# saholmes/stark-mlwe

Measured on AMD Instinct MI355X. Metric: prove ms + Fr-NTT achieved GB/s, 2^20/2^24 trace at 1/2/4/8 GPUs, higher is better.
Workload: dtype u256 (4x u64 Montgomery limbs, Pallas Fr); 1 GPU; one 2^20-row trace x 4 columns (2^20 rows per GPU), blowup 8: LDE (iNTT + coset NTT) + DEEP-ALI merge + FRI folds + Poseidon leaf hashes + Poseidon-Merkle trees (schedule [16,16,8]), kernels only; log_trace_per_gpu=20, log_blowup=3, field=pallas_fr

## Files before the change

### stark_mlwe_amd/csrc/capi_core.hip

```cpp
#include <algorithm>
#include <cstring>
#include "poseidon_launch.hpp"
#include "pow_table.hpp"

using namespace stark;

namespace stark {

static int32_t pool_poison_fill(stark_ctx* ctx, void* p, size_t bytes) {
    STARK_HIP(ctx, hipMemsetAsync(p, ctx->opt.pool_poison, bytes, ctx->stream));
    STARK_HIP(ctx, hipStreamSynchronize(ctx->stream));
    return STARK_OK;
}

int32_t ctx_scratch(stark_ctx* ctx, size_t bytes, void** out) {
    if (bytes > ctx->scratch_bytes) {
        if (ctx->scratch) STARK_HIP(ctx, hipStreamSynchronize(ctx->stream));
        ctx->scratch_bytes = 0; STARK_HIP(ctx, ctx->scratch.alloc(bytes)); ctx->scratch_bytes = bytes;
    }
    if (ctx->opt.pool_poison >= 0 && ctx->scratch_bytes) STARK_TRY(pool_poison_fill(ctx, ctx->scratch.p, ctx->scratch_bytes));
    *out = ctx->scratch.p; return STARK_OK;
}

int32_t ctx_upload_staged(stark_ctx* ctx, void* dst, const void* src, size_t bytes) {
    if (!bytes) return STARK_OK;
    auto& q = ctx->staged;
    for (size_t i = 0; i < q.size();) {
        if (hipEventQuery(q[i].done) == hipSuccess) { (void)hipEventDestroy(q[i].done); q[i] = std::move(q.back()); q.pop_back(); } else ++i;
    }
    (void)hipGetLastError();
    stark_ctx::StagedUpload u; u.host.reset(new uint8_t[bytes]); memcpy(u.host.get(), src, bytes);
    STARK_HIP(ctx, hipEventCreateWithFlags(&u.done, hipEventDisableTiming));
    const uint8_t* from = u.host.get();
    q.push_back(std::move(u));
    STARK_HIP(ctx, hipMemcpyAsync(dst, from, bytes, hipMemcpyHostToDevice, ctx->stream));
    STARK_HIP(ctx, hipEventRecord(q.back().done, ctx->stream));
    return STARK_OK;
}

static inline size_t pool_round(size_t bytes) {
    if (bytes < 256) return 256;
    if (bytes <= (1u << 20)) { size_t r = 256; while (r < bytes) r <<= 1; return r; }
    return (bytes + (1u << 20) - 1) & ~(size_t)((1u << 20) - 1);
}
int32_t ctx_alloc(stark_ctx* ctx, size_t bytes, void** out) {
    const size_t sz = pool_round(bytes);
    auto it = ctx->pool_free.find(sz);
    if (it != ctx->pool_free.end() && !it->second.empty()) {
        void* p = it->second.back(); it->second.pop_back(); ctx->pool_cached_bytes -= sz;
        ctx->pool_live[p] = sz; *out = p;
        return ctx->opt.pool_poison >= 0 ? pool_poison_fill(ctx, p, sz) : STARK_OK;
    }
    void* p = nullptr; hipError_t e = hipMalloc(&p, sz);
    if (e != hipSuccess) {
        (void)hipGetLastError();
        (void)hipStreamSynchronize(ctx->stream);
        for (auto& kv : ctx->pool_free) { for (void* q : kv.second) (void)hipFree(q); kv.second.clear(); }
        ctx->pool_cached_bytes = 0;
        e = hipMalloc(&p, sz);
        if (e != hipSuccess) { (void)hipGetLastError(); return ctx->fail(STARK_ERR_OOM, "device allocation of " + std::to_string(sz) + " bytes failed"); }
    }
    ctx->pool_live[p] = sz; *out = p;
    return ctx->opt.pool_poison >= 0 ? pool_poison_fill(ctx, p, sz) : STARK_OK;
}
void ctx_release(stark_ctx* ctx, void* p) {
    if (!p || !ctx) return;
    auto it = ctx->pool_live.find(p);
    if (it == ctx->pool_live.end()) { ctx->err = "ctx_release: the pointer is not a live block of this context's pool (left alone)"; return; }
    const size_t sz = it->second; ctx->pool_live.erase(it);
    ctx->pool_free[sz].push_back(p); ctx->pool_cached_bytes += sz;
}
int32_t ctx_enter(stark_ctx* ctx) {
    if (!ctx) return STARK_ERR_INVALID_ARG;
    int cur = -1;
    if (hipGetDevice(&cur) != hipSuccess || cur != ctx->device) STARK_HIP(ctx, hipSetDevice(ctx->device));
    return STARK_OK;
}

int32_t ctx_side_stream(stark_ctx* ctx, hipStream_t* out) {
    if (!ctx->side_stream) { STARK_HIP(ctx, hipStreamCreateWithFlags(&ctx->side_stream, hipStreamNonBlocking)); STARK_HIP(ctx, hipEventCreateWithFlags(&ctx->ev_fork, hipEventDisableTiming)); }
    *out = ctx->side_stream; return STARK_OK;
}
int32_t ctx_fork(stark_ctx* ctx, hipStream_t* side) {
    STARK_TRY(ctx_side_stream(ctx, side));
    if (hipEventRecord(ctx->ev_fork, ctx->stream) != hipSuccess || hipStreamWaitEvent(*side, ctx->ev_fork, 0) != hipSuccess) return ctx->fail(STARK_ERR_HIP, "fork");
    return STARK_OK;
}
int32_t ctx_join(stark_ctx* ctx) {
    if (hipEventRecord(ctx->ev_fork, ctx->side_stream) != hipSuccess || hipStreamWaitEvent(ctx->stream, ctx->ev_fork, 0) != hipSuccess) return ctx->fail(STARK_ERR_HIP, "join");
    return STARK_OK;
}

static int32_t params_finish(stark_ctx* ctx, stark_params* P) {
    if (host::rp_for_width(P->ref.t) < 0) return ctx->fail(STARK_ERR_UNSUPPORTED, "Poseidon width must be one of 9,17,33,65,129");
    P->kc = host::make_kernel_consts(P->ref);
    if (!P->kc.ok) return ctx->fail(STARK_ERR_UNSUPPORTED, "MDS matrix has a singular leading minor: LU/sparse kernel form unavailable");
    const host::KernelConsts& k = P->kc;
    std::vector<fr_t> blob; auto put = [&](const std::vector<fr_t>& v) { size_t off = blob.size(); blob.insert(blob.end(), v.begin(), v.end()); return off; };
    size_t o_rcf = put(k.rc_full), o_rcp = put(k.rc_partial), o_lu = put(k.lu), o_pre = put(k.lu_pre), o_row0 = put(k.row0), o_sp = put(k.sparse), o_mds = put(k.mds), o_mpre = put(k.mds_pre), o_gam = put(k.gamma);
    const size_t o_29 = blob.size();
    { std::vector<uint32_t> w29; for (auto* v : {&k.lu29, &k.lu_pre29, &k.row0_29, &k.sparse29, &k.gamma29, &k.mds29, &k.mds_pre29, &k.chain_a, &k.chain_g, &k.chain_w}) w29.insert(w29.end(), v->begin(), v->end());
      while (w29.size() % 8) w29.push_back(0);
      blob.resize(o_29 + w29.size() / 8); memcpy((void*)(blob.data() + o_29), w29.data(), w29.size() * 4); }
    const size_t o_frag = blob.size(), frag_elems = (k.mds_frag.size() + sizeof(fr_t) - 1) / sizeof(fr_t);
    if (!k.mds_frag.empty()) { blob.resize(o_frag + 2 * frag_elems); memcpy((void*)(blob.data() + o_frag), k.mds_frag.data(), k.mds_frag.size()); memcpy((void*)(blob.data() + o_frag + frag_elems), k.mds_pre_frag.data(), k.mds_pre_frag.size()); }
    const size_t o_b8 = blob.size(), ef_elems = (k.blk8_efrag.size() + sizeof(fr_t) - 1) / sizeof(fr_t), lf_elems = (k.blk8_lfrag.size() + sizeof(fr_t) - 1) / sizeof(fr_t), gf_elems = (k.blk8_gfrag.size() + sizeof(fr_t) - 1) / sizeof(fr_t);
    if (!k.blk8_efrag.empty()) { blob.resize(o_b8 + ef_elems + lf_elems + gf_elems); memcpy((void*)(blob.data() + o_b8), k.blk8_efrag.data(), k.blk8_efrag.size()); memcpy((void*)(blob.data() + o_b8 + ef_elems), k.blk8_lfrag.data(), k.blk8_lfrag.size());
                                 memcpy((void*)(blob.data() + o_b8 + ef_elems + lf_elems), k.blk8_gfrag.data(), k.blk8_gfrag.size()); }
    STARK_HIP(ctx, P->blob.alloc(blob.size() * sizeof(fr_t)));
    fr_t* const dev = P->blob.fr();
    STARK_HIP(ctx, hipMemcpyAsync(dev, blob.data(), blob.size() * sizeof(fr_t), hipMemcpyHostToDevice, ctx->stream));
    STARK_HIP(ctx, hipStreamSynchronize(ctx->stream));
    P->dev.t = k.t; P->dev.rf = k.rf; P->dev.rp = k.rp;
    P->dev.rc_full = dev + o_rcf; P->dev.rc_partial = dev + o_rcp; P->dev.lu = dev + o_lu; P->dev.lu_pre = dev + o_pre;
    P->dev.row0 = dev + o_row0; P->dev.sparse = dev + o_sp; P->dev.mds = dev + o_mds; P->dev.mds_pre = dev + o_mpre; P->dev.gamma = dev + o_gam;
    { const uint32_t* b29 = reinterpret_cast<const uint32_t*>(dev + o_29);
      P->dev.lu29 = b29; P->dev.lu_pre29 = b29 + k.lu29.size(); P->dev.row0_29 = P->dev.lu_pre29 + k.lu_pre29.size();
      P->dev.sparse29 = P->dev.row0_29 + k.row0_29.size(); P->dev.gamma29 = P->dev.sparse29 + k.sparse29.size();
      P->dev.mds29 = P->dev.gamma29 + k.gamma29.size(); P->dev.mds_pre29 = P->dev.mds29 + k.mds29.size();
      const uint32_t* ch = P->dev.mds_pre29 + k.mds_pre29.size();
      P->dev.chain_a = k.chain_a.empty() ? nullptr : ch; P->dev.chain_g = k.chain_a.empty() ? nullptr : ch + k.chain_a.size(); P->dev.chain_w = k.chain_a.empty() ? nullptr : ch + k.chain_a.size() + k.chain_g.size(); }
    P->dev.blk8_efrag = k.blk8_efrag.empty() ? nullptr : (const void*)(dev + o_b8); P->dev.blk8_lfrag = k.blk8_efrag.empty() ? nullptr : (const void*)(dev + o_b8 + ef_elems);
    P->dev.blk8_gfrag = k.blk8_gfrag.empty() ? nullptr : (const void*)(dev + o_b8 + ef_elems + lf_elems);
    P->dev.blk8_unit_frag = k.blk8_efrag.empty() ? nullptr : (const void*)((const int8_t*)P->dev.blk8_lfrag + k.blk8_lfrag.size() - 1024);
    P->dev.mds_frag = k.mds_frag.empty() ? nullptr : (const void*)(dev + o_frag); P->dev.mds_pre_frag = k.mds_frag.empty() ? nullptr : (const void*)(dev + o_frag + frag_elems);
    return STARK_OK;
}
static int32_t params_from_consts(stark_ctx* ctx, const host::PoseidonConsts& c, std::unique_ptr<stark_params>& out) {
    std::unique_ptr<stark_params> P(new stark_params()); P->ctx = ctx; P->ref = c;
    STARK_TRY(params_finish(ctx, P.get()));
    out = std::move(P); return STARK_OK;
}
static int32_t params_for_caller(stark_ctx* ctx, const host::PoseidonConsts& c, stark_params** out) {
    std::unique_ptr<stark_params> P; STARK_TRY(params_from_consts(ctx, c, P));
    P->ref_.bind(ctx); *out = P.release(); return STARK_OK;
}
int32_t ctx_transcript_params(stark_ctx* ctx, stark_params** out) {
    if (!ctx->tparams) STARK_TRY(params_from_consts(ctx, host::consts_transcript(), ctx->tparams));
    if (out) *out = ctx->tparams.get();
    return STARK_OK;
}
int32_t ctx_merkle_params(stark_ctx* ctx, int t, stark_params** out) {
    auto it = ctx->merkle_params.find(t);
    if (it == ctx->merkle_params.end()) {
        if (host::rp_for_width(t) < 0) return ctx->fail(STARK_ERR_UNSUPPORTED, "unsupported Poseidon width");
        std::unique_ptr<stark_params> P; STARK_TRY(params_from_consts(ctx, host::consts_for_width(t), P));
        *out = P.get(); ctx->merkle_params[t] = std::move(P); return STARK_OK;
    }
    *out = it->second.get(); return STARK_OK;
}
int32_t ctx_commit_params(stark_ctx* ctx, stark_params** out) {
    std::unique_ptr<stark_params>& slot = ctx->merkle_params[-17];
    if (!slot) STARK_TRY(params_from_consts(ctx, host::derive_consts("POSEIDON-T17-X5-SEED", 17, 8, 64), slot));
    *out = slot.get(); return STARK_OK;
}

}

extern "C" {

int32_t stark_version(void) { return 1; }

int32_t stark_ctx_create(int32_t device, void* stream, stark_ctx_t** out) {
    if (!out) return STARK_ERR_INVALID_ARG;
    int ndev = 0;
    if (hipGetDeviceCount(&ndev) != hipSuccess || ndev <= 0 || device < 0 || device >= ndev) return STARK_ERR_HIP;
    if (hipSetDevice(device) != hipSuccess) return STARK_ERR_HIP;
    std::unique_ptr<stark_ctx> c(new stark_ctx()); c->device = device;
    if (stream == STARK_STREAM_PRIVATE) { if (hipStreamCreateWithFlags(&c->stream, hipStreamNonBlocking) != hipSuccess) return STARK_ERR_HIP; c->own_stream = true; }
    else { c->stream = (hipStream_t)stream; c->own_stream = false; }
    if (hipEventCreate(&c->ev0) != hipSuccess || hipEventCreate(&c->ev1) != hipSuccess) return STARK_ERR_HIP;
    { int cus = 0; if (hipDeviceGetAttribute(&cus, hipDeviceAttributeMultiprocessorCount, device) == hipSuccess && cus > 0) c->num_cus = cus; }
    stark::ntt_set_attrs();
    stark::poseidon_set_attrs();
    *out = c.release(); return STARK_OK;
}
}
static void ctx_teardown(stark_ctx* ctx) {
    (void)hipSetDevice(ctx->device); (void)hipStreamSynchronize(ctx->stream);
    stark::comm_destroy(ctx);
    stark::ntt_plans_free(ctx);
    for (auto& kv : ctx->pool_free) for (void* q : kv.second) (void)hipFree(q);
    for (auto& kv : ctx->pool_live) (void)hipFree(kv.first);
    if (ctx->pinned) (void)hipHostFree(ctx->pinned);
    for (auto& u : ctx->staged) (void)hipEventDestroy(u.done);
    if (ctx->ev0) (void)hipEventDestroy(ctx->ev0); if (ctx->ev1) (void)hipEventDestroy(ctx->ev1);
    if (ctx->side_stream) (void)hipStreamDestroy(ctx->side_stream);
    if (ctx->ev_fork) (void)hipEventDestroy(ctx->ev_fork);
    if (ctx->own_stream) (void)hipStreamDestroy(ctx->stream);
    delete ctx;
}
namespace stark {
void ctx_ref(stark_ctx* c) { ++c->live_handles; }
void ctx_unref(stark_ctx* c) { if (--c->live_handles == 0 && c->destroy_pending) ctx_teardown(c); }
}
extern "C" {
int32_t stark_ctx_destroy(stark_ctx_t* ctx) {
    if (!ctx) return STARK_ERR_INVALID_ARG;
    if (ctx->destroy_pending) return STARK_ERR_INVALID_ARG;
    STARK_TRY(ctx_enter(ctx));
    (void)hipStreamSynchronize(ctx->stream);
    if (ctx->live_handles > 0) { ctx->destroy_pending = true; return STARK_OK; }
    ctx_teardown(ctx); return STARK_OK;
}
int32_t stark_ctx_sync(stark_ctx_t* ctx) { if (!ctx) return STARK_ERR_INVALID_ARG; STARK_TRY(ctx_enter(ctx)); STARK_HIP(ctx, hipStreamSynchronize(ctx->stream)); return STARK_OK; }
int32_t stark_ctx_trim(stark_ctx_t* ctx) {
    if (!ctx) return STARK_ERR_INVALID_ARG; STARK_TRY(ctx_enter(ctx));
    STARK_HIP(ctx, hipStreamSynchronize(ctx->stream));
    for (auto& kv : ctx->pool_free) { for (void* q : kv.second) (void)hipFree(q); kv.second.clear(); }
    ctx->pool_cached_bytes = 0;
    stark::ntt_plans_free(ctx);
    ctx->scratch.reset(); ctx->scratch_bytes = 0;
    return STARK_OK;
}
size_t stark_ctx_cached_bytes(stark_ctx_t* ctx) { return ctx ? ctx->pool_cached_bytes : 0; }
}
struct OptionDef { const char* key; const char* (*set)(stark_ctx::Options&, int64_t); };
static const OptionDef kOptions[] = {
    {"ntt_direct_max_log", [](stark_ctx::Options& o, int64_t v) -> const char* { if (v < 0 || v > 30) return "0..30"; o.ntt_direct_max_log = (int)v; return nullptr; }},
    {"ntt_merged_coset", [](stark_ctx::Options& o, int64_t v) -> const char* { o.ntt_merged_coset = v != 0; return nullptr; }},
    {"ntt_log_tile", [](stark_ctx::Options& o, int64_t v) -> const char* { if (v != -1 && (v < 8 || v > 12)) return "8..12, or -1 for the default"; o.ntt_log_tile_forced = v != -1; o.ntt_log_tile = v == -1 ? 11 : (int)v; return nullptr; }},
    {"ntt_min_waves", [](stark_ctx::Options& o, int64_t v) -> const char* { if (v != 2 && v != 4) return "2 or 4"; o.ntt_min_waves = (int)v; return nullptr; }},
    {"poseidon_lane_only", [](stark_ctx::Options& o, int64_t v) -> const char* { o.poseidon_lane_only = v != 0; return nullptr; }},
    {"sponge_one_wave", [](stark_ctx::Options& o, int64_t v) -> const char* { o.sponge_one_wave = v != 0; return nullptr; }},
    {"sponge_debug", [](stark_ctx::Options& o, int64_t v) -> const char* { o.sponge_debug = (int)v; return nullptr; }},
    {"merkle_node16_pair", [](stark_ctx::Options& o, int64_t v) -> const char* { o.merkle_node16_pair = v != 0; return nullptr; }},
    {"poseidon_block8", [](stark_ctx::Options& o, int64_t v) -> const char* { o.poseidon_block8 = v != 0; return nullptr; }},
    {"fri_side_pair", [](stark_ctx::Options& o, int64_t v) -> const char* { o.fri_side_pair = v != 0; return nullptr; }},
    {"sumcheck_verify_batch_max_slots", [](stark_ctx::Options& o, int64_t v) -> const char* { if (v < 1) return "at least 1"; o.sumcheck_verify_batch_max_slots = (size_t)v; return nullptr; }},
    {"ntt_batch_max_elems", [](stark_ctx::Options& o, int64_t v) -> const char* { if (v < 1 || v > ((int64_t)1 << 28)) return "1..2^28"; o.ntt_batch_max_elems = (size_t)v; return nullptr; }},
    {"prove_batch_max_rows", [](stark_ctx::Options& o, int64_t v) -> const char* { if (v < 1 || v > ((int64_t)1 << 28)) return "1..2^28"; o.prove_batch_max_rows = (size_t)v; return nullptr; }},
    {"mle_log_tile", [](stark_ctx::Options& o, int64_t v) -> const char* { if (v != -1 && (v < 3 || v > 12)) return "3..12, or -1 for the default"; o.mle_log_tile = (int)v; return nullptr; }},
    {"mle_lane_contiguous", [](stark_ctx::Options& o, int64_t v) -> const char* { if (v < -1 || v > 1) return "0 or 1, or -1 for the default"; o.mle_lane_contiguous = (int)v; return nullptr; }},
    {"lagrange_max_partials", [](stark_ctx::Options& o, int64_t v) -> const char* { if (v != -1 && (v < 1 || v > ((int64_t)1 << 28))) return "1..2^28, or -1 for the default"; o.lagrange_max_partials = v == -1 ? (size_t)1 << 21 : (size_t)v; return nullptr; }},
    {"lagrange_wide_acc", [](stark_ctx::Options& o, int64_t v) -> const char* { if (v < -1 || v > 1) return "0 or 1, or -1 for the default"; o.lagrange_wide_acc = (int)v; return nullptr; }},
    {"pool_poison", [](stark_ctx::Options& o, int64_t v) -> const char* { if (v < -1 || v > 255) return "0..255, or -1 for off"; o.pool_poison = (int)v; return nullptr; }},
};
extern "C" {
int32_t stark_ctx_set_option(stark_ctx_t* ctx, const char* key, int64_t value) {
    if (!ctx || !key) return STARK_ERR_INVALID_ARG;
    STARK_TRY(ctx_enter(ctx));
    const std::string k(key);
    const OptionDef* def = nullptr; std::string known;
    for (const OptionDef& d : kOptions) { if (k == d.key) def = &d; known += (known.empty() ? "" : ", ") + std::string(d.key); }
    if (!def) return ctx->fail(STARK_ERR_INVALID_ARG, "unknown option '" + k + "' (" + known + ")");
    if (const char* range = def->set(ctx->opt, value)) return ctx->fail(STARK_ERR_INVALID_ARG, k + ": " + range);
    STARK_HIP(ctx, hipStreamSynchronize(ctx->stream));
    stark::ntt_plans_free(ctx);
    return STARK_OK;
}
const char* stark_last_error(stark_ctx_t* ctx) { return ctx ? ctx->err.c_str() : "null context"; }
int32_t stark_malloc(stark_ctx_t* ctx, size_t bytes, void** dptr) { if (!ctx || !dptr) return STARK_ERR_INVALID_ARG; STARK_TRY(ctx_enter(ctx)); STARK_HIP(ctx, hipMalloc(dptr, bytes ? bytes : 32)); return STARK_OK; }
int32_t stark_free(stark_ctx_t* ctx, void* dptr) { if (!ctx) return STARK_ERR_INVALID_ARG; STARK_TRY(ctx_enter(ctx)); STARK_HIP(ctx, hipStreamSynchronize(ctx->stream)); STARK_HIP(ctx, hipFree(dptr)); return STARK_OK; }
int32_t stark_memcpy_h2d(stark_ctx_t* ctx, void* d, const void* s, size_t bytes) {
    if (!ctx) return STARK_ERR_INVALID_ARG;
    STARK_TRY(ctx_enter(ctx));
    STARK_HIP(ctx, hipMemcpyAsync(d, s, bytes, hipMemcpyHostToDevice, ctx->stream)); STARK_HIP(ctx, hipStreamSynchronize(ctx->stream)); return STARK_OK; }
int32_t stark_memcpy_d2h(stark_ctx_t* ctx, void* d, const void* s, size_t bytes) {
    if (!ctx) return STARK_ERR_INVALID_ARG;
    STARK_TRY(ctx_enter(ctx));
    STARK_HIP(ctx, hipMemcpyAsync(d, s, bytes, hipMemcpyDeviceToHost, ctx->stream)); STARK_HIP(ctx, hipStreamSynchronize(ctx->stream)); return STARK_OK; }
int32_t stark_timer_start(stark_ctx_t* ctx) { if (!ctx) return STARK_ERR_INVALID_ARG; STARK_HIP(ctx, hipEventRecord(ctx->ev0, ctx->stream)); return STARK_OK; }
int32_t stark_timer_stop_ms(stark_ctx_t* ctx, float* ms) {
    if (!ctx || !ms) return STARK_ERR_INVALID_ARG;
    STARK_TRY(ctx_enter(ctx));
    STARK_HIP(ctx, hipEventRecord(ctx->ev1, ctx->stream)); STARK_HIP(ctx, hipEventSynchronize(ctx->ev1)); STARK_HIP(ctx, hipEventElapsedTime(ms, ctx->ev0, ctx->ev1)); return STARK_OK; }

}
#define STARK_DIAG_ITERS 2048
static __global__ void __launch_bounds__(1024) k_diag_mac_rate(uint32_t* out, uint32_t seed) {
    uint32_t a0 = seed + threadIdx.x, a1 = a0 * 3 + 1, a2 = a0 * 5 + 2, a3 = a0 * 7 + 3, a4 = a0 * 9 + 4, a5 = a0 * 11 + 5, a6 = a0 * 13 + 6, a7 = a0 * 15 + 7;
    uint64_t d0 = a0, d1 = a1, d2 = a2, d3 = a3, d4 = a4, d5 = a5, d6 = a6, d7 = a7; const uint32_t b = seed | 1;
#define STARK_DIAG_MAD(i) asm volatile("v_mad_u64_u32 %0, vcc, %1, %2, %0" : "+v"(d##i) : "v"(a##i), "v"(b) : "vcc");
    for (int i = 0; i < STARK_DIAG_ITERS; ++i) { STARK_DIAG_MAD(0) STARK_DIAG_MAD(1) STARK_DIAG_MAD(2) STARK_DIAG_MAD(3) STARK_DIAG_MAD(4) STARK_DIAG_MAD(5) STARK_DIAG_MAD(6) STARK_DIAG_MAD(7) }
#undef STARK_DIAG_MAD
    out[blockIdx.x * blockDim.x + threadIdx.x] = (uint32_t)(d0 ^ d1 ^ d2 ^ d3 ^ d4 ^ d5 ^ d6 ^ d7);
}
extern "C" {
int32_t stark_diag_mac_rate(stark_ctx_t* ctx, double* lane_macs_per_s) {
    if (!ctx || !lane_macs_per_s) return STARK_ERR_INVALID_ARG;
    STARK_TRY(ctx_enter(ctx));
    hipDeviceProp_t prop; STARK_HIP(ctx, hipGetDeviceProperties(&prop, ctx->device));
    const int blocks = prop.multiProcessorCount * 2, threads = 1024;
    DevBuf o; STARK_HIP(ctx, o.alloc(ctx, (size_t)blocks * threads * 4));
    hipLaunchKernelGGL(k_diag_mac_rate, dim3(blocks), dim3(threads), 0, ctx->stream, (uint32_t*)o.p, 12345u);
    STARK_HIP(ctx, hipEventRecord(ctx->ev0, ctx->stream));
    hipLaunchKernelGGL(k_diag_mac_rate, dim3(blocks), dim3(threads), 0, ctx->stream, (uint32_t*)o.p, 12345u);
    STARK_HIP(ctx, hipGetLastError());
    STARK_HIP(ctx, hipEventRecord(ctx->ev1, ctx->stream)); STARK_HIP(ctx, hipEventSynchronize(ctx->ev1));
    float ms = 0; STARK_HIP(ctx, hipEventElapsedTime(&ms, ctx->ev0, ctx->ev1));
    *lane_macs_per_s = (double)blocks * threads * 8.0 * STARK_DIAG_ITERS / (ms * 1e-3);
    return STARK_OK;
}

int32_t stark_poseidon_params_upload(stark_ctx_t* ctx, int32_t t, int32_t rf, int32_t rp, const uint64_t* mds, const uint64_t* rc_full, const uint64_t* rc_partial, stark_params_t** out) {
    if (!ctx || !mds || !rc_full || !rc_partial || !out || t < 2 || rf <= 0 || (rf & 1) || rp <= 0) return ctx ? ctx->fail(STARK_ERR_INVALID_ARG, "bad params") : STARK_ERR_INVALID_ARG;
    STARK_TRY(ctx_enter(ctx));
    host::PoseidonConsts c; c.t = t; c.rf = rf; c.rp = rp;
    c.mds.resize((size_t)t * t); c.rc_full.resize((size_t)rf * t); c.rc_partial.resize(rp);
    for (size_t i = 0; i < c.mds.size(); ++i) c.mds[i] = load_fr(mds + 4 * i);
    for (size_t i = 0; i < c.rc_full.size(); ++i) c.rc_full[i] = load_fr(rc_full + 4 * i);
    for (size_t i = 0; i < c.rc_partial.size(); ++i) c.rc_partial[i] = load_fr(rc_partial + 4 * i);
    return params_for_caller(ctx, c, out);
}
int32_t stark_poseidon_params_for_width(stark_ctx_t* ctx, int32_t t, stark_params_t** out) {
    if (!ctx || !out) return STARK_ERR_INVALID_ARG;
    STARK_TRY(ctx_enter(ctx));
    if (host::rp_for_width(t) < 0) return ctx->fail(STARK_ERR_UNSUPPORTED, "unsupported Poseidon width t; supported t in {9,17,33,65,129}");
    return params_for_caller(ctx, host::consts_for_width(t), out);
}
int32_t stark_poseidon_params_t17_seed(stark_ctx_t* ctx, const uint8_t* seed, size_t n, stark_params_t** out) {
    if (!ctx || !out || (!seed && n)) return STARK_ERR_INVALID_ARG;
    STARK_TRY(ctx_enter(ctx));
    return params_for_caller(ctx, host::derive_consts(std::string((const char*)seed, n), 17, 8, 64), out);
}
int32_t stark_poseidon_params_export(stark_params_t* p, int32_t* t, int32_t* rf, int32_t* rp, uint64_t* mds, uint64_t* rc_full, uint64_t* rc_partial) {
    if (!p) return STARK_ERR_INVALID_ARG;
    if (t) *t = p->ref.t; if (rf) *rf = p->ref.rf; if (rp) *rp = p->ref.rp;
    if (mds) for (size_t i = 0; i < p->ref.mds.size(); ++i) store_fr(mds + 4 * i, p->ref.mds[i]);
    if (rc_full) for (size_t i = 0; i < p->ref.rc_full.size(); ++i) store_fr(rc_full + 4 * i, p->ref.rc_full[i]);
    if (rc_partial) for (size_t i = 0; i < p->ref.rc_partial.size(); ++i) store_fr(rc_partial + 4 * i, p->ref.rc_partial[i]);
    return STARK_OK;
}
int32_t stark_poseidon_params_free(stark_params_t* p) { if (!p) return STARK_ERR_INVALID_ARG; delete p; return STARK_OK; }

}
```

### stark_mlwe_amd/csrc/host_util.hpp

```cpp
#pragma once
#include <cstdint>
#include <cstring>
#include <string>
#include <vector>
#include "fr.hpp"
#include "fr29.hpp"

namespace stark {
namespace host {

struct Blake3 {
    static constexpr uint32_t kIV[8] = {0x6A09E667u, 0xBB67AE85u, 0x3C6EF372u, 0xA54FF53Au, 0x510E527Fu, 0x9B05688Cu, 0x1F83D9ABu, 0x5BE0CD19u};
    enum : uint32_t { F_CHUNK_START = 1, F_CHUNK_END = 2, F_PARENT = 4, F_ROOT = 8 };
    static uint32_t ror(uint32_t x, unsigned n) { return (x >> n) | (x << (32 - n)); }
    static void mix(uint32_t* v, int a, int b, int c, int d, uint32_t x, uint32_t y) {
        v[a] += v[b] + x; v[d] = ror(v[d] ^ v[a], 16); v[c] += v[d]; v[b] = ror(v[b] ^ v[c], 12);
        v[a] += v[b] + y; v[d] = ror(v[d] ^ v[a], 8);  v[c] += v[d]; v[b] = ror(v[b] ^ v[c], 7);
    }
    static void compress(const uint32_t h[8], const uint8_t block[64], uint32_t blen, uint64_t ctr, uint32_t flags, uint32_t out[16]) {
        static const uint8_t sched[7][16] = {
            {0, 1, 2, 3, 4, 5, 6, 7, 8, 9, 10, 11, 12, 13, 14, 15}, {2, 6, 3, 10, 7, 0, 4, 13, 1, 11, 12, 5, 9, 14, 15, 8},
            {3, 4, 10, 12, 13, 2, 7, 14, 6, 5, 9, 0, 11, 15, 8, 1}, {10, 7, 12, 9, 14, 3, 13, 15, 4, 0, 11, 2, 5, 8, 1, 6},
            {12, 13, 9, 11, 15, 10, 14, 8, 7, 2, 5, 3, 0, 1, 6, 4}, {9, 14, 11, 5, 8, 12, 15, 1, 13, 3, 0, 10, 2, 6, 4, 7},
            {11, 15, 5, 0, 1, 9, 8, 6, 14, 10, 2, 12, 3, 4, 7, 13}};
        uint32_t m[16], v[16];
        for (int i = 0; i < 16; ++i) m[i] = (uint32_t)block[4 * i] | (uint32_t)block[4 * i + 1] << 8 | (uint32_t)block[4 * i + 2] << 16 | (uint32_t)block[4 * i + 3] << 24;
        for (int i = 0; i < 8; ++i) v[i] = h[i];
        for (int i = 0; i < 4; ++i) v[8 + i] = kIV[i];
        v[12] = (uint32_t)ctr; v[13] = (uint32_t)(ctr >> 32); v[14] = blen; v[15] = flags;
        for (int r = 0; r < 7; ++r) {
            const uint8_t* s = sched[r];
            mix(v, 0, 4, 8, 12, m[s[0]], m[s[1]]);   mix(v, 1, 5, 9, 13, m[s[2]], m[s[3]]);
            mix(v, 2, 6, 10, 14, m[s[4]], m[s[5]]);  mix(v, 3, 7, 11, 15, m[s[6]], m[s[7]]);
            mix(v, 0, 5, 10, 15, m[s[8]], m[s[9]]);  mix(v, 1, 6, 11, 12, m[s[10]], m[s[11]]);
            mix(v, 2, 7, 8, 13, m[s[12]], m[s[13]]); mix(v, 3, 4, 9, 14, m[s[14]], m[s[15]]);
        }
        for (int i = 0; i < 8; ++i) { out[i] = v[i] ^ v[i + 8]; out[i + 8] = v[i + 8] ^ h[i]; }
    }
    struct Node { uint32_t h[8]; uint8_t block[64]; uint32_t blen; uint64_t ctr; uint32_t flags; };
    static void cv_of(const Node& n, uint32_t extra, uint32_t cv[8]) { uint32_t o[16]; compress(n.h, n.block, n.blen, n.ctr, n.flags | extra, o); memcpy(cv, o, 32); }
    static Node chunk_node(const uint8_t* p, size_t len, uint64_t index) {
        Node n; memcpy(n.h, kIV, 32); n.ctr = index;
        size_t off = 0; bool first = true;
        while (len - off > 64) {
            uint32_t o[16]; compress(n.h, p + off, 64, index, first ? F_CHUNK_START : 0, o); memcpy(n.h, o, 32);
            off += 64; first = false;
        }
        memset(n.block, 0, 64); memcpy(n.block, p + off, len - off); n.blen = (uint32_t)(len - off);
        n.flags = (first ? F_CHUNK_START : 0) | F_CHUNK_END;
        return n;
    }
    static Node subtree(const uint8_t* p, size_t len, uint64_t index) {
        if (len <= 1024) return chunk_node(p, len, index);
        size_t chunks = (len + 1023) / 1024, left = 1; while (left * 2 < chunks) left *= 2;
        Node l = subtree(p, left * 1024, index), r = subtree(p + left * 1024, len - left * 1024, index + left);
        Node n; memcpy(n.h, kIV, 32); n.ctr = 0; n.blen = 64; n.flags = F_PARENT;
        uint32_t a[8], b[8]; cv_of(l, 0, a); cv_of(r, 0, b);
        for (int i = 0; i < 8; ++i) for (int j = 0; j < 4; ++j) { n.block[4 * i + j] = (uint8_t)(a[i] >> (8 * j)); n.block[32 + 4 * i + j] = (uint8_t)(b[i] >> (8 * j)); }
        return n;
    }
    static void hash(const uint8_t* p, size_t len, uint8_t out[32]) {
        Node root = subtree(p, len, 0);
        if (root.flags & F_PARENT) root.ctr = 0;
        uint32_t cv[8]; cv_of(root, F_ROOT, cv);
        for (int i = 0; i < 8; ++i) for (int j = 0; j < 4; ++j) out[4 * i + j] = (uint8_t)(cv[i] >> (8 * j));
    }
};

struct ChaCha12Rng {
    uint32_t st[16]; uint32_t out[16]; unsigned have = 0;
    explicit ChaCha12Rng(const uint8_t seed[32]) {
        st[0] = 0x61707865u; st[1] = 0x3320646eu; st[2] = 0x79622d32u; st[3] = 0x6b206574u;
        for (int i = 0; i < 8; ++i) st[4 + i] = (uint32_t)seed[4 * i] | (uint32_t)seed[4 * i + 1] << 8 | (uint32_t)seed[4 * i + 2] << 16 | (uint32_t)seed[4 * i + 3] << 24;
        st[12] = st[13] = st[14] = st[15] = 0;
    }
    static uint32_t rol(uint32_t x, unsigned n) { return (x << n) | (x >> (32 - n)); }
    void block() {
        uint32_t x[16]; memcpy(x, st, 64);
        auto Q = [&](int a, int b, int c, int d) {
            x[a] += x[b]; x[d] = rol(x[d] ^ x[a], 16); x[c] += x[d]; x[b] = rol(x[b] ^ x[c], 12);
            x[a] += x[b]; x[d] = rol(x[d] ^ x[a], 8);  x[c] += x[d]; x[b] = rol(x[b] ^ x[c], 7); };
        for (int i = 0; i < 6; ++i) { Q(0, 4, 8, 12); Q(1, 5, 9, 13); Q(2, 6, 10, 14); Q(3, 7, 11, 15); Q(0, 5, 10, 15); Q(1, 6, 11, 12); Q(2, 7, 8, 13); Q(3, 4, 9, 14); }
        for (int i = 0; i < 16; ++i) out[i] = x[i] + st[i];
        if (++st[12] == 0) ++st[13];
        have = 16;
    }
    uint32_t next_u32() { if (!have) block(); return out[16 - have--]; }
    uint64_t next_u64() { uint64_t lo = next_u32(), hi = next_u32(); return lo | hi << 32; }
};

typedef PallasFr PF;
inline fr_t h_one() { return fr_one<PF>(); }
inline fr_t h_zero() { return fr_zero<PF>(); }
inline fr_t h_mul(const fr_t& a, const fr_t& b) { return fr_mul<PF>(a, b); }
inline fr_t h_add(const fr_t& a, const fr_t& b) { return fr_add<PF>(a, b); }
inline fr_t h_sub(const fr_t& a, const fr_t& b) { return fr_sub<PF>(a, b); }
inline fr_t h_u64(uint64_t x) { return fr_from_u64<PF>(x); }
inline fr_t h_from_le_bytes_mod_order(const uint8_t* b, size_t n) {
    fr_t acc = h_zero(); const fr_t two32 = h_u64(1ull << 32);
    size_t nw = (n + 3) / 4;
    for (size_t k = nw; k-- > 0;) {
        uint32_t w = 0; for (size_t j = 0; j < 4; ++j) if (4 * k + j < n) w |= (uint32_t)b[4 * k + j] << (8 * j);
        acc = h_add(h_mul(acc, two32), h_u64(w));
    }
    return acc;
}
inline void h_to_bytes_le(const fr_t& a, uint8_t out[32]) {
    fr_t c = fr_to_canonical<PF>(a);
    for (int i = 0; i < 8; ++i) for (int j = 0; j < 4; ++j) out[4 * i + j] = (uint8_t)(c.v[i] >> (8 * j));
}
inline fr_t h_fr_from_hash(const char* tag, const std::vector<uint8_t>& data) {
    std::vector<uint8_t> buf(tag, tag + strlen(tag)); buf.insert(buf.end(), data.begin(), data.end());
    uint8_t d[32]; Blake3::hash(buf.data(), buf.size(), d);
    uint8_t wide[64]; memset(wide, 0, 64); memcpy(wide, d, 32);
    return h_from_le_bytes_mod_order(wide, 64);
}
inline fr_t h_tag(const char* s) {
    size_t n = strlen(s);
    if (n <= 32) { uint8_t le[32] = {0}; memcpy(le, s, n); return h_from_le_bytes_mod_order(le, 32); }
    fr_t acc = h_zero();
    for (size_t off = 0; off < n; off += 32) { uint8_t le[32] = {0}; size_t c = n - off < 32 ? n - off : 32; memcpy(le, s + off, c); acc = h_add(acc, h_from_le_bytes_mod_order(le, 32)); }
    return acc;
}
inline std::vector<fr_t> h_words(const char* s) {
    std::vector<fr_t> out; size_t n = strlen(s);
    for (size_t off = 0; off < n; off += 31) { uint8_t le[32] = {0}; size_t c = n - off < 31 ? n - off : 31; memcpy(le, s + off, c); out.push_back(h_from_le_bytes_mod_order(le, 32)); }
    return out;
}
inline int tr_hash_frame(const char* tag, std::vector<fr_t>& frame) {
    const fr_t AB = h_tag("FSv1-ABSORB-BYTES"), CH = h_tag("FSv1-CHALLENGE");
    frame.clear();
    frame.push_back(AB); for (auto& w : h_words("FRI/FS")) frame.push_back(w);
    frame.push_back(AB); for (auto& w : h_words(tag)) frame.push_back(w);
    const int np = (int)frame.size();
    frame.push_back(CH); frame.push_back(AB); for (auto& w : h_words("out")) frame.push_back(w);
    return np;
}

struct PoseidonConsts {
    int t = 0, rf = 0, rp = 0;
    std::vector<fr_t> mds;
    std::vector<fr_t> rc_full;
    std::vector<fr_t> rc_partial;
};
inline void put64(std::vector<uint8_t>& v, uint64_t x) { for (int j = 0; j < 8; ++j) v.push_back((uint8_t)(x >> (8 * j))); }
inline PoseidonConsts derive_consts(const std::string& seed, int t, int rf, int rp) {
    PoseidonConsts c; c.t = t; c.rf = rf; c.rp = rp;
    c.mds.resize((size_t)t * t); c.rc_full.resize((size_t)rf * t); c.rc_partial.resize(rp);
    for (int i = 0; i < t; ++i) for (int j = 0; j < t; ++j) { std::vector<uint8_t> d; put64(d, i); put64(d, j); d.insert(d.end(), seed.begin(), seed.end()); c.mds[(size_t)i * t + j] = h_fr_from_hash("POSEIDON-MDS", d); }
    for (int r = 0; r < rf; ++r) for (int i = 0; i < t; ++i) { std::vector<uint8_t> d; put64(d, r); put64(d, i); d.insert(d.end(), seed.begin(), seed.end()); c.rc_full[(size_t)r * t + i] = h_fr_from_hash("POSEIDON-RC-FULL", d); }
    for (int r = 0; r < rp; ++r) { std::vector<uint8_t> d; put64(d, r); d.insert(d.end(), seed.begin(), seed.end()); c.rc_partial[r] = h_fr_from_hash("POSEIDON-RC-PART", d); }
    return c;
}
inline int width_for_arity(size_t arity) { return arity <= 8 ? 9 : arity <= 16 ? 17 : arity <= 32 ? 33 : arity <= 64 ? 65 : arity <= 128 ? 129 : -1; }
inline int rp_for_width(int t) { switch (t) { case 9: return 60; case 17: return 64; case 33: return 68; case 65: return 76; case 129: return 84; default: return -1; } }
inline PoseidonConsts consts_for_width(int t) {
    std::string seed = "POSEIDON-PALLAS-T"; for (int j = 0; j < 8; ++j) seed.push_back((char)(((uint64_t)t >> (8 * j)) & 0xff));
    return derive_consts(seed, t, 8, rp_for_width(t));
}
inline PoseidonConsts consts_transcript() { return derive_consts("POSEIDON-T17-X5-TRANSCRIPT", 17, 8, 64); }

struct KernelConsts {
    int t = 0, rf = 0, rp = 0;
    std::vector<fr_t> rc_full, rc_partial;
    std::vector<fr_t> lu, lu_pre;
    std::vector<fr_t> row0;
    std::vector<fr_t> sparse;
    std::vector<fr_t> mds;
    std::vector<fr_t> mds_pre;
    std::vector<fr_t> gamma;
    std::vector<uint32_t> lu29, lu_pre29, row0_29, sparse29, gamma29;
    std::vector<uint32_t> mds29, mds_pre29;
    std::vector<int8_t> mds_frag, mds_pre_frag;
    std::vector<uint32_t> chain_a, chain_g, chain_w;
    std::vector<int8_t> blk8_efrag, blk8_lfrag, blk8_gfrag;
    std::vector<uint32_t> gamma8_29;
    bool ok = false;
};
template <class Pred> inline std::vector<uint32_t> to_radix29(const std::vector<fr_t>& v, Pred scaled) {
    const fr_t k = fr_from_u64<PF>(1ull << FR29_SBOX_SHIFT);
    std::vector<uint32_t> o(v.size() * 9);
    for (size_t i = 0; i < v.size(); ++i) fr29_const_from<PF>(scaled(i) ? fr_mul<PF>(v[i], k) : v[i], &o[9 * i]);
    return o;
}
inline void mfma_frag_of(fr_t g, int8_t* out) {
    const fr_t k256 = fr_from_u64<PF>(256);
    int8_t d[32][32];
    for (int b = 0; b < 32; ++b, g = h_mul(g, k256)) {
        const fr_t c = fr_to_canonical<PF>(g); int cy = 0;
        for (int k = 0; k < 32; ++k) { const int v = (int)((c.v[k >> 2] >> (8 * (k & 3))) & 0xff) + 0x80 + cy; cy = v >> 8; d[b][k] = (int8_t)((v & 0xff) - 0x80); }
    }
    for (int l = 0; l < 64; ++l) for (int j = 0; j < 16; ++j) out[(size_t)l * 16 + j] = d[16 * (l >> 5) + j][l & 31];
}
inline std::vector<int8_t> mfma_frags(const fr_t* mat, int rows, int cols, const fr_t& scale) {
    std::vector<int8_t> out((size_t)rows * cols * 64 * 16, 0);
    for (int i = 0; i < rows; ++i) for (int e = 0; e < cols; ++e) mfma_frag_of(h_mul(mat[(size_t)i * cols + e], scale), &out[((size_t)i * cols + e) * 64 * 16]);
    return out;
}
inline std::vector<int8_t> mfma_frags(const std::vector<fr_t>& mat, int t) { return mfma_frags(mat.data(), t, t, fr_from_u64<PF>(1ull << FR29_SBOX_SHIFT)); }
inline bool mat_inverse(std::vector<fr_t> a, int n, std::vector<fr_t>& inv) {
    inv.assign((size_t)n * n, h_zero()); for (int i = 0; i < n; ++i) inv[(size_t)i * n + i] = h_one();
    for (int c = 0; c < n; ++c) {
        int p = -1; for (int r = c; r < n; ++r) if (!fr_is_zero(a[(size_t)r * n + c])) { p = r; break; }
        if (p < 0) return false;
        if (p != c) for (int k = 0; k < n; ++k) { std::swap(a[(size_t)p * n + k], a[(size_t)c * n + k]); std::swap(inv[(size_t)p * n + k], inv[(size_t)c * n + k]); }
        fr_t pi = fr_inv<PF>(a[(size_t)c * n + c]);
        for (int k = 0; k < n; ++k) { a[(size_t)c * n + k] = h_mul(a[(size_t)c * n + k], pi); inv[(size_t)c * n + k] = h_mul(inv[(size_t)c * n + k], pi); }
        for (int r = 0; r < n; ++r) if (r != c) {
            fr_t f = a[(size_t)r * n + c]; if (fr_is_zero(f)) continue;
            for (int k = 0; k < n; ++k) { a[(size_t)r * n + k] = h_sub(a[(size_t)r * n + k], h_mul(f, a[(size_t)c * n + k])); inv[(size_t)r * n + k] = h_sub(inv[(size_t)r * n + k], h_mul(f, inv[(size_t)c * n + k])); }
        }
    }
    return true;
}
inline bool lu_pack(const std::vector<fr_t>& m, int n, std::vector<fr_t>& lu) {
    lu = m;
    for (int k = 0; k < n; ++k) {
        if (fr_is_zero(lu[(size_t)k * n + k])) return false;
        fr_t pi = fr_inv<PF>(lu[(size_t)k * n + k]);
        for (int i = k + 1; i < n; ++i) {
            fr_t f = h_mul(lu[(size_t)i * n + k], pi); lu[(size_t)i * n + k] = f;
            for (int j = k + 1; j < n; ++j) lu[(size_t)i * n + j] = h_sub(lu[(size_t)i * n + j], h_mul(f, lu[(size_t)k * n + j]));
        }
    }
    return true;
}
inline KernelConsts make_kernel_consts(const PoseidonConsts& c) {
    KernelConsts k; k.t = c.t; k.rf = c.rf; k.rp = c.rp; k.rc_full = c.rc_full; k.rc_partial = c.rc_partial; k.mds = c.mds;
    const int t = c.t, n = t - 1;
    k.row0.assign(c.mds.begin(), c.mds.begin() + t);
    std::vector<fr_t> cur = c.mds;
    k.sparse.assign((size_t)c.rp * (2 * t - 1), h_zero());
    for (int r = c.rp - 1; r >= 0; --r) {
        std::vector<fr_t> hat((size_t)n * n), hinv;
        for (int i = 0; i < n; ++i) for (int j = 0; j < n; ++j) hat[(size_t)i * n + j] = cur[(size_t)(i + 1) * t + (j + 1)];
        if (!mat_inverse(hat, n, hinv)) return k;
        fr_t* sp = &k.sparse[(size_t)r * (2 * t - 1)];
        sp[0] = cur[0];
        for (int j = 0; j < n; ++j) { fr_t acc = h_zero(); for (int q = 0; q < n; ++q) acc = h_add(acc, h_mul(cur[(size_t)0 * t + (q + 1)], hinv[(size_t)q * n + j])); sp[1 + j] = acc; }
        for (int i = 0; i < n; ++i) sp[t + i] = cur[(size_t)(i + 1) * t + 0];
        std::vector<fr_t> nxt((size_t)t * t);
        for (int j = 0; j < t; ++j) nxt[j] = c.mds[j];
        for (int i = 0; i < n; ++i) for (int j = 0; j < t; ++j) { fr_t acc = h_zero(); for (int q = 0; q < n; ++q) acc = h_add(acc, h_mul(hat[(size_t)i * n + q], c.mds[(size_t)(q + 1) * t + j])); nxt[(size_t)(i + 1) * t + j] = acc; }
        cur.swap(nxt);
    }
    if (c.rp % 4) return k;
    k.gamma.assign((size_t)(c.rp / 4) * 6, h_zero());
    for (int b = 0; b < c.rp / 4; ++b)
        for (int q = 1; q < 4; ++q)
            for (int p2 = 0; p2 < q; ++p2) {
                const fr_t* uq = &k.sparse[(size_t)(4 * b + q) * (2 * t - 1)];
                const fr_t* wp = &k.sparse[(size_t)(4 * b + p2) * (2 * t - 1)];
                fr_t acc = h_zero();
                for (int j = 1; j < t; ++j) acc = h_add(acc, h_mul(uq[j], wp[t - 1 + j]));
                k.gamma[(size_t)b * 6 + q * (q - 1) / 2 + p2] = acc;
            }
    if (!lu_pack(c.mds, t, k.lu)) return k;
    if (!lu_pack(cur, t, k.lu_pre)) return k;
    k.mds_pre = cur;
    const auto upper = [t](size_t i) { return (int)(i % t) >= (int)(i / t); };
    const auto all = [](size_t) { return true; };
    const auto a_and_w = [t](size_t i) { const int c = (int)(i % (2 * t - 1)); return c == 0 || c >= t; };
    k.lu29 = to_radix29(k.lu, upper); k.lu_pre29 = to_radix29(k.lu_pre, upper); k.row0_29 = to_radix29(k.row0, all);
    k.sparse29 = to_radix29(k.sparse, a_and_w); k.gamma29 = to_radix29(k.gamma, all);
    k.mds29 = to_radix29(k.mds, all); k.mds_pre29 = to_radix29(k.mds_pre, all);
    if (t == 17) { k.mds_frag = mfma_frags(k.mds, t); k.mds_pre_frag = mfma_frags(k.mds_pre, t); }
    if (t == 17 && c.rp % 8 == 0) {
        const int nb = c.rp / 8, w = 2 * t - 1;
        const fr_t s20 = fr_from_u64<PF>(1ull << FR29_SBOX_SHIFT);
        std::vector<fr_t> g8((size_t)nb * 28, h_zero()), um((size_t)8 * n), wm((size_t)n * 8);
        for (int b = 0; b < nb; ++b) {
            for (int q = 0; q < 8; ++q) for (int j = 1; j < t; ++j) {
                um[(size_t)q * n + (j - 1)] = k.sparse[(size_t)(8 * b + q) * w + j];
                wm[(size_t)(j - 1) * 8 + q] = k.sparse[(size_t)(8 * b + q) * w + t - 1 + j];
            }
            const std::vector<int8_t> ef = mfma_frags(um.data(), 8, n, h_one()), lf = mfma_frags(wm.data(), n, 8, s20);
            k.blk8_efrag.insert(k.blk8_efrag.end(), ef.begin(), ef.end()); k.blk8_lfrag.insert(k.blk8_lfrag.end(), lf.begin(), lf.end());
            for (int q = 1; q < 8; ++q) for (int p2 = 0; p2 < q; ++p2) {
                fr_t acc = h_zero();
                for (int j = 0; j < n; ++j) acc = h_add(acc, h_mul(um[(size_t)q * n + j], wm[(size_t)j * 8 + p2]));
                g8[(size_t)b * 28 + q * (q - 1) / 2 + p2] = acc;
                k.blk8_gfrag.resize(k.blk8_gfrag.size() + 1024); mfma_frag_of(h_mul(acc, s20), &k.blk8_gfrag[k.blk8_gfrag.size() - 1024]);
            }
        }
        k.blk8_lfrag.resize(k.blk8_lfrag.size() + 1024); mfma_frag_of(h_one(), &k.blk8_lfrag[k.blk8_lfrag.size() - 1024]);
        k.gamma8_29 = to_radix29(g8, all);
    }
    if (t == 17 && c.rp == 64) {
        const int rp = c.rp, w = 2 * t - 1;
        const fr_t scale = fr_from_u64<PF>(1ull << 25);
        auto limbs = [&](const fr_t& v, uint32_t* out) { const fr29_t u = fr29_unpack(h_mul(v, scale)); for (int i = 0; i < 9; ++i) out[i] = u.l[i]; };
        k.chain_a.assign((size_t)rp * 64, 0u); k.chain_g.assign((size_t)rp * 9 * 64, 0u); k.chain_w.assign((size_t)rp * (t - 1) * 9, 0u);
        for (int q = 0; q < rp; ++q) {
            uint32_t l[9]; limbs(k.sparse[(size_t)q * w], l);
            for (int i = 0; i < 9; ++i) k.chain_a[(size_t)q * 64 + 16 + i] = l[i];
            for (int j = 1; j < t; ++j) limbs(k.sparse[(size_t)q * w + t - 1 + j], &k.chain_w[((size_t)q * (t - 1) + (j - 1)) * 9]);
        }
        for (int q = 1; q < rp; ++q)
            for (int p2 = 0; p2 < q; ++p2) {
                const fr_t* uq = &k.sparse[(size_t)q * w]; const fr_t* wp = &k.sparse[(size_t)p2 * w];
                fr_t acc = h_zero();
                for (int j = 1; j < t; ++j) acc = h_add(acc, h_mul(uq[j], wp[t - 1 + j]));
                uint32_t l[9]; limbs(acc, l);
                if (q == p2 + 1) { for (int i = 0; i < 9; ++i) k.chain_a[(size_t)p2 * 64 + 32 + i] = l[i]; }
                else for (int i = 0; i < 9; ++i) k.chain_g[((size_t)p2 * 9 + i) * 64 + q] = l[i];
            }
    }
    k.ok = true;
    return k;
}

inline void permute_dense(fr_t* s, const PoseidonConsts& c) {
    const int t = c.t, half = c.rf / 2; std::vector<fr_t> o(t);
    auto mds = [&]() { for (int i = 0; i < t; ++i) { fr_t acc = h_zero(); for (int j = 0; j < t; ++j) acc = h_add(acc, h_mul(c.mds[(size_t)i * t + j], s[j])); o[i] = acc; } for (int i = 0; i < t; ++i) s[i] = o[i]; };
    for (int r = 0; r < half; ++r) { for (int i = 0; i < t; ++i) s[i] = fr_pow5<PF>(h_add(s[i], c.rc_full[(size_t)r * t + i])); mds(); }
    for (int r = 0; r < c.rp; ++r) { s[0] = fr_pow5<PF>(h_add(s[0], c.rc_partial[r])); mds(); }
    for (int r = half; r < c.rf; ++r) { for (int i = 0; i < t; ++i) s[i] = fr_pow5<PF>(h_add(s[i], c.rc_full[(size_t)r * t + i])); mds(); }
}

}
}
```

### stark_mlwe_amd/csrc/hostcheck.cpp

```cpp
#include <algorithm>
#include <atomic>
#include <cstring>
#include <vector>
#include "fr.hpp"
#include "host_util.hpp"
#include "poseidon_dev.hpp"
#include "fri_plan.hpp"
#include "fri_verify.hpp"
#include "fri_verify_batch.hpp"
#include "mfma_digits.hpp"
#include "poseidon_chain.hpp"
#include "fri_batch.hpp"
#include "ntt_batch_plan.hpp"
#include "sumcheck_impl.hpp"
#include "mle_dev.hpp"
#include "merkle_batch.hpp"
#include "lagrange_dev.hpp"

using namespace stark;

static fr_t ld4(const uint64_t* p) { fr_t x; for (int i = 0; i < 4; ++i) { x.v[2 * i] = (uint32_t)p[i]; x.v[2 * i + 1] = (uint32_t)(p[i] >> 32); } return x; }
static void st4(uint64_t* p, const fr_t& x) { for (int i = 0; i < 4; ++i) p[i] = (uint64_t)x.v[2 * i] | ((uint64_t)x.v[2 * i + 1] << 32); }

static int g_alloc_fill = 0;
static std::vector<uint64_t> hc_block(size_t bytes) { std::vector<uint64_t> v((bytes + 7) / 8 + 1); memset(v.data(), g_alloc_fill, v.size() * sizeof(uint64_t)); return v; }
static std::vector<fr_t> hc_fr_block(size_t n) { std::vector<fr_t> v(n); if (n) memset((void*)v.data(), g_alloc_fill, n * sizeof(fr_t)); return v; }

struct HcParams { host::PoseidonConsts ref; host::KernelConsts kc; PoseidonDev dev; };
static void bind(HcParams* P) {
    P->kc = host::make_kernel_consts(P->ref);
    P->dev.t = P->kc.t; P->dev.rf = P->kc.rf; P->dev.rp = P->kc.rp; P->dev.rc_full = P->kc.rc_full.data(); P->dev.rc_partial = P->kc.rc_partial.data();
    P->dev.lu = P->kc.lu.data(); P->dev.lu_pre = P->kc.lu_pre.data(); P->dev.row0 = P->kc.row0.data(); P->dev.sparse = P->kc.sparse.data(); P->dev.mds = P->kc.mds.data(); P->dev.mds_pre = P->kc.mds_pre.data(); P->dev.gamma = P->kc.gamma.data();
    P->dev.lu29 = P->kc.lu29.data(); P->dev.lu_pre29 = P->kc.lu_pre29.data(); P->dev.row0_29 = P->kc.row0_29.data(); P->dev.sparse29 = P->kc.sparse29.data(); P->dev.gamma29 = P->kc.gamma29.data(); P->dev.mds29 = P->kc.mds29.data(); P->dev.mds_pre29 = P->kc.mds_pre29.data();
    P->dev.mds_frag = nullptr; P->dev.mds_pre_frag = nullptr; P->dev.blk8_efrag = nullptr; P->dev.blk8_lfrag = nullptr; P->dev.blk8_unit_frag = nullptr; P->dev.blk8_gfrag = nullptr;
    P->dev.chain_a = P->kc.chain_a.empty() ? nullptr : P->kc.chain_a.data(); P->dev.chain_g = P->kc.chain_g.empty() ? nullptr : P->kc.chain_g.data(); P->dev.chain_w = P->kc.chain_w.empty() ? nullptr : P->kc.chain_w.data();
}

extern "C" {

int hc_set_alloc_fill(int byte) { if (byte < 0 || byte > 255) return -1; const int old = g_alloc_fill; g_alloc_fill = byte; return old; }
int hc_alloc_probe(size_t bytes, uint8_t* out) { const std::vector<uint64_t> v = hc_block(bytes); memcpy(out, v.data(), bytes); return 0; }

int hc_fr_op(int field, int op, const uint64_t* a, const uint64_t* b, uint64_t* out) {
    fr_t x = ld4(a), y = b ? ld4(b) : x, z;
    if (field == 0) {
        switch (op) { case 0: z = fr_add<PallasFr>(x, y); break; case 1: z = fr_sub<PallasFr>(x, y); break; case 2: z = fr_mul<PallasFr>(x, y); break; case 3: z = fr_inv<PallasFr>(x); break;
            case 4: z = fr_from_u64<PallasFr>(a[0]); break; case 5: z = fr_to_canonical<PallasFr>(x); break; case 6: z = fr_root_of_unity<PallasFr>((unsigned)a[0]); break;
            case 7: z = fr_pow_u64<PallasFr>(x, b[0]); break; case 8: z = fr_pow5_r29<PallasFr>(x); break; default: return -1; }
    } else {
        switch (op) { case 0: z = fr_add<Bls12381Fr>(x, y); break; case 1: z = fr_sub<Bls12381Fr>(x, y); break; case 2: z = fr_mul<Bls12381Fr>(x, y); break; case 3: z = fr_inv<Bls12381Fr>(x); break;
            case 4: z = fr_from_u64<Bls12381Fr>(a[0]); break; case 5: z = fr_to_canonical<Bls12381Fr>(x); break; case 6: z = fr_root_of_unity<Bls12381Fr>((unsigned)a[0]); break;
            case 7: z = fr_pow_u64<Bls12381Fr>(x, b[0]); break; case 8: z = fr_pow5_r29<Bls12381Fr>(x); break; default: return -1; }
    }
    st4(out, z); return 0;
}
int hc_wide_dot(const uint64_t* a, const uint64_t* b, size_t n, uint64_t* out) {
    DotAcc d; d.init();
    for (size_t i = 0; i < n; ++i) { uint32_t c[9]; fr29_const_from<PF>(ld4(a + 4 * i), c); d.mac(c, ld4(b + 4 * i)); }
    st4(out, d.finish()); return 0;
}
int hc_wide_dot32(const uint64_t* a, const uint64_t* b, size_t n, uint64_t* out) {
    if (n > 24) return -1;
    fr_wide w; fr_wide_zero(w);
    for (size_t i = 0; i < n; ++i) fr_wide_mac_f<PF>(w, ld4(a + 4 * i), ld4(b + 4 * i));
    st4(out, fr_wide_reduce<PF>(w)); return 0;
}
}
template <class F> static int hc_ntt29_impl(uint64_t* data, int log_b, int inverse, uint64_t* max_limb, uint64_t* max_top) {
    if (log_b < 1 || log_b > 16) return -1;
    const size_t B = (size_t)1 << log_b;
    fr_t w = fr_root_of_unity<F>((unsigned)log_b); if (inverse) w = fr_inv<F>(w);
    const fr_t k32 = fr_from_u64<F>(32);
    std::vector<fr29_t> tw(B / 2), x(B);
    { fr_t acc = k32; for (size_t i = 0; i < B / 2; ++i) { tw[i] = fr29_unpack(acc); acc = fr_mul<F>(acc, w); } }
    uint32_t D[9]; ntt29_offset<F>(D);
    auto brev = [&](size_t v) { size_t r = 0; for (int i = 0; i < log_b; ++i) r |= ((v >> i) & 1) << (log_b - 1 - i); return r; };
    for (size_t p = 0; p < B; ++p) x[brev(p)] = fr29_unpack(ld4(data + 4 * p));
    uint64_t ml = 0, mt = 0;
    const int head = log_b >= 3 ? 3 : log_b;
    {
        const fr29_t w1 = tw[log_b >= 3 ? B >> 3 : 0], w2 = tw[log_b >= 2 ? B >> 2 : 0], w3 = tw[log_b >= 3 ? 3 * (B >> 3) : 0];
        for (size_t g = 0; g < (B >> head); ++g) {
            fr29_t* xs = &x[g << head];
            if (head == 3) ntt29_head<F, 3>(*reinterpret_cast<fr29_t (*)[8]>(xs), w1, w2, w3, D);
            else if (head == 2) ntt29_head<F, 2>(*reinterpret_cast<fr29_t (*)[4]>(xs), w1, w2, w3, D);
            else ntt29_head<F, 1>(*reinterpret_cast<fr29_t (*)[2]>(xs), w1, w2, w3, D);
        }
    }
    for (int s = head + 1; s <= log_b; ++s) {
        const size_t half = (size_t)1 << (s - 1); const bool nrm = ntt29_norm_before(s);
        for (size_t bq = 0; bq < B / 2; ++bq) {
            const size_t j = bq & (half - 1), grp = bq >> (s - 1), i0 = (grp << s) + j, i1 = i0 + half;
            fr29_t a = x[i0], b = x[i1];
            { fr29_t bb = b, aa = a; if (nrm) { fr29_norm(bb); fr29_norm(aa); } for (int k = 0; k < 8; ++k) { ml = std::max<uint64_t>(ml, bb.l[k]); ml = std::max<uint64_t>(ml, aa.l[k]); } mt = std::max<uint64_t>(mt, std::max(bb.l[8], aa.l[8])); }
            ntt29_butterfly<F>(a, b, tw[j << (log_b - s)], D, nrm);
            x[i0] = a; x[i1] = b;
        }
    }
    const bool nrm_out = ntt29_norm_after(log_b);
    fr_t mult = k32; if (inverse) mult = fr_mul<F>(k32, fr_inv<F>(fr_from_u64<F>((uint64_t)B)));
    for (size_t k = 0; k < B; ++k) {
        fr29_t y = x[k];
        for (int i = 0; i < 8; ++i) ml = std::max<uint64_t>(ml, nrm_out ? 0 : y.l[i]);
        if (inverse) {
            if (nrm_out) fr29_norm(y);
            mt = std::max<uint64_t>(mt, y.l[8]);
            const fr29_t r = fr29_mul_mont<F>(fr29_unpack(mult), y);
            st4(data + 4 * k, fr29_pack_reduce<F>(r.l));
        } else {
            fr29_partial_reduce<F>(y);
            st4(data + 4 * k, fr29_pack_reduce<F>(y.l));
        }
    }
    if (max_limb) *max_limb = ml; if (max_top) *max_top = mt;
    return 0;
}
extern "C" {
int hc_partial_reduce(int field, uint32_t* limbs, size_t n) {
    for (size_t i = 0; i < n; ++i) {
        fr29_t x; for (int k = 0; k < 9; ++k) x.l[k] = limbs[9 * i + k];
        if (field == 0) fr29_partial_reduce<PallasFr>(x); else fr29_partial_reduce<Bls12381Fr>(x);
        for (int k = 0; k < 9; ++k) limbs[9 * i + k] = x.l[k];
    }
    return 0;
}
int hc_ntt29(int field, uint64_t* data, int log_b, int inverse, uint64_t* max_limb, uint64_t* max_top) {
    return field == 0 ? hc_ntt29_impl<PallasFr>(data, log_b, inverse, max_limb, max_top) : hc_ntt29_impl<Bls12381Fr>(data, log_b, inverse, max_limb, max_top);
}
int hc_blake3(const uint8_t* p, size_t n, uint8_t* out32) { host::Blake3::hash(p, n, out32); return 0; }
int hc_chacha12_u64s(const uint8_t* seed32, size_t n, uint64_t* out) { host::ChaCha12Rng r(seed32); for (size_t i = 0; i < n; ++i) out[i] = r.next_u64(); return 0; }
int hc_from_le_bytes_mod_order(const uint8_t* b, size_t n, uint64_t* out) { st4(out, host::h_from_le_bytes_mod_order(b, n)); return 0; }
int hc_to_bytes_le(const uint64_t* a, uint8_t* out32) { host::h_to_bytes_le(ld4(a), out32); return 0; }

void* hc_params_new(int kind, int t, const char* seed) {
    HcParams* P = new HcParams();
    P->ref = kind == 0 ? host::consts_for_width(t) : kind == 1 ? host::consts_transcript() : host::derive_consts(seed, 17, 8, 64);
    bind(P); return P;
}
void* hc_params_upload(int t, int rf, int rp, const uint64_t* mds, const uint64_t* rc_full, const uint64_t* rc_partial) {
    if (!mds || !rc_full || !rc_partial || t < 2 || rf <= 0 || (rf & 1) || rp <= 0) return nullptr;
    HcParams* P = new HcParams();
    P->ref.t = t; P->ref.rf = rf; P->ref.rp = rp;
    P->ref.mds.resize((size_t)t * t); P->ref.rc_full.resize((size_t)rf * t); P->ref.rc_partial.resize(rp);
    for (size_t i = 0; i < P->ref.mds.size(); ++i) P->ref.mds[i] = ld4(mds + 4 * i);
    for (size_t i = 0; i < P->ref.rc_full.size(); ++i) P->ref.rc_full[i] = ld4(rc_full + 4 * i);
    for (size_t i = 0; i < P->ref.rc_partial.size(); ++i) P->ref.rc_partial[i] = ld4(rc_partial + 4 * i);
    bind(P); return P;
}
int hc_params_ok(void* h) { return ((HcParams*)h)->kc.ok ? 1 : 0; }
void hc_params_free(void* h) { delete (HcParams*)h; }
int hc_params_export(void* h, uint64_t* mds, uint64_t* rc_full, uint64_t* rc_partial) {
    HcParams* P = (HcParams*)h;
    for (size_t i = 0; i < P->ref.mds.size(); ++i) st4(mds + 4 * i, P->ref.mds[i]);
    for (size_t i = 0; i < P->ref.rc_full.size(); ++i) st4(rc_full + 4 * i, P->ref.rc_full[i]);
    for (size_t i = 0; i < P->ref.rc_partial.size(); ++i) st4(rc_partial + 4 * i, P->ref.rc_partial[i]);
    return 0;
}
int hc_full_round_linear(void* h, int which, int pre, uint64_t* states, size_t n) {
    HcParams* P = (HcParams*)h; const int t = P->dev.t;
    if (t != 17 || P->kc.mds_frag.empty()) return -1;
    std::vector<fr_t> st(t), out(t);
    const std::vector<int8_t>& F = pre ? P->kc.mds_pre_frag : P->kc.mds_frag;
    for (size_t s = 0; s < n; ++s) {
        for (int j = 0; j < t; ++j) st[j] = ld4(states + 4 * (s * t + j));
        if (which == 0) { ArrayState a{st.data()}; apply_lu(a, pre ? P->dev.lu_pre29 : P->dev.lu29, t); out = st; }
        else {
            std::vector<fr_t> xd(t); for (int e = 0; e < t; ++e) xd[e] = recode_signed(st[e]);
            for (int i = 0; i < t; ++i) {
                int32_t S[32];
                for (int r = 0; r < 32; ++r) { int64_t acc = 0;
                    for (int e = 0; e < t; ++e) for (int kh = 0; kh < 2; ++kh) { const int8_t* a = &F[((((size_t)i * t + e) * 64) + (r + 32 * kh)) * 16];
                        const int8_t* b = reinterpret_cast<const int8_t*>(xd[e].v) + 16 * kh; for (int j = 0; j < 16; ++j) acc += (int64_t)a[j] * b[j]; }
                    if (acc > 0x7fffffffll || acc < -0x80000000ll) return -2; S[r] = (int32_t)acc; }
                int32_t lo[16], hi[16];
                for (int reg = 0; reg < 16; ++reg) { const int row = (reg & 3) + 8 * (reg >> 2); lo[reg] = S[row]; hi[reg] = S[row + 4]; }
                int64_t col[9]; for (int k = 0; k < 9; ++k) col[k] = 0;
                mfma_fold_rows(col, lo, hi);
                out[i] = mfma_finish_cols(col);
            }
        }
        for (int j = 0; j < t; ++j) st4(states + 4 * (s * t + j), out[j]);
    }
    return 0;
}
size_t hc_mfma_frag_table(void* h, int pre, int8_t* out, size_t cap) {
    HcParams* P = (HcParams*)h; const std::vector<int8_t>& F = pre ? P->kc.mds_pre_frag : P->kc.mds_frag;
    if (out) memcpy(out, F.data(), std::min(cap, F.size()));
    return F.size();
}
int hc_mfma_finish(const int32_t* sums, size_t n, uint64_t* out) {
    for (size_t s = 0; s < n; ++s) {
        const int32_t* S = sums + 32 * s;
        for (int c = 0; c < 32; ++c) if (S[c] >= (1 << 24) || S[c] <= -(1 << 24)) return -1;
        int32_t lo[16], hi[16];
        for (int reg = 0; reg < 16; ++reg) { const int row = (reg & 3) + 8 * (reg >> 2); lo[reg] = S[row]; hi[reg] = S[row + 4]; }
        int64_t col[9]; for (int k = 0; k < 9; ++k) col[k] = 0;
        mfma_fold_rows(col, lo, hi);
        st4(out + 4 * s, mfma_finish_cols(col));
    }
    return 0;
}
static int blk8_tile_sums(const int8_t* const* frag, const fr_t* xd, int K, int32_t* S) {
    for (int r = 0; r < 32; ++r) { int64_t acc = 0;
        for (int k = 0; k < K; ++k) for (int kh = 0; kh < 2; ++kh) { const int8_t* a = frag[k] + (size_t)(r + 32 * kh) * 16;
            const int8_t* b = reinterpret_cast<const int8_t*>(xd[k].v) + 16 * kh; for (int j = 0; j < 16; ++j) acc += (int64_t)a[j] * b[j]; }
        if (acc >= (1 << 24) || acc <= -(1 << 24)) return -2; S[r] = (int32_t)acc; }
    return 0;
}
static fr_t blk8_finish_sums(const int32_t* S) {
    int32_t lo[16], hi[16];
    for (int reg = 0; reg < 16; ++reg) { const int row = (reg & 3) + 8 * (reg >> 2); lo[reg] = S[row]; hi[reg] = S[row + 4]; }
    int64_t col[9]; for (int k = 0; k < 9; ++k) col[k] = 0;
    mfma_fold_rows(col, lo, hi);
    return mfma_finish_cols(col);
}
static int blk8_tile(const int8_t* const* frag, const fr_t* xd, int K, fr_t& out) { int32_t S[32]; const int rc = blk8_tile_sums(frag, xd, K, S); if (rc) return rc; out = blk8_finish_sums(S); return 0; }
static std::atomic<int32_t> g_blk8_row23_max{0};
int32_t hc_blk8_row23_max(int reset) { return reset ? g_blk8_row23_max.exchange(0) : g_blk8_row23_max.load(); }
int hc_permute_block8(void* h, uint64_t* states, size_t n) {
    HcParams* P = (HcParams*)h; const host::KernelConsts& k = P->kc; const int t = k.t, half = k.rf / 2, W = 2 * t - 1;
    if (t != 17 || k.blk8_efrag.empty() || k.blk8_gfrag.empty() || k.mds_frag.empty()) return -1;
    const int8_t* unit = k.blk8_lfrag.data() + k.blk8_lfrag.size() - 1024;
    std::vector<fr_t> st(t), xd(t), o(t);
    auto full = [&](int r, const std::vector<int8_t>& F) -> int {
        for (int j = 0; j < t; ++j) xd[j] = recode_signed(fr_pow5_r29<PF>(fr_add<PF>(st[j], k.rc_full[(size_t)r * t + j])));
        for (int i = 0; i < t; ++i) { const int8_t* fr[17]; for (int e = 0; e < t; ++e) fr[e] = &F[((size_t)i * t + e) * 1024]; const int rc = blk8_tile(fr, xd.data(), t, o[i]); if (rc) return rc; }
        st = o; return 0; };
    for (size_t s = 0; s < n; ++s) {
        for (int j = 0; j < t; ++j) st[j] = ld4(states + 4 * (s * t + j));
        for (int r = 0; r < half; ++r) { const int rc = full(r, r == half - 1 ? k.mds_pre_frag : k.mds_frag); if (rc) return rc; }
        fr_t s0 = st[0], rec[17], y[8], yd[9], kx[23];
        for (int j = 1; j < t; ++j) rec[j] = recode_signed(st[j]);
        const int nb = k.rp / 8;
        for (int b = 0; b < nb; ++b) {
            const int8_t* ef = k.blk8_efrag.data() + (size_t)b * 8 * 16 * 1024; const int8_t* lf = k.blk8_lfrag.data() + (size_t)b * 16 * 8 * 1024;
            const int8_t* gf = k.blk8_gfrag.data() + (size_t)b * 28 * 1024;
            for (int j = 0; j < 16; ++j) kx[j] = rec[1 + j];
            for (int q = 0; q < 8; ++q) {
                const int8_t* fr[23]; for (int j = 0; j < 16; ++j) fr[j] = ef + ((size_t)q * 16 + j) * 1024;
                for (int p2 = 0; p2 < q; ++p2) { fr[16 + p2] = gf + ((size_t)q * (q - 1) / 2 + p2) * 1024; kx[16 + p2] = yd[p2]; }
                int32_t S[32]; { const int rc = blk8_tile_sums(fr, kx, 16 + q, S); if (rc) return rc; }
                if (q == 7) { int32_t m = 0; for (int c = 0; c < 32; ++c) m = std::max(m, S[c] < 0 ? -S[c] : S[c]);
                              int32_t seen = g_blk8_row23_max.load(); while (m > seen && !g_blk8_row23_max.compare_exchange_weak(seen, m)) {} }
                const fr_t H = blk8_finish_sums(S);
                y[q] = fr_pow5_r29<PF>(fr_add<PF>(s0, k.rc_partial[8 * b + q]));
                yd[q] = recode_signed(y[q]);
                DotAcc acc; acc.init();
                acc.mac(c29(k.sparse29.data(), (size_t)(8 * b + q) * W), y[q]);
                s0 = fr_add<PF>(H, acc.finish());
            }
            for (int j = 1; j < t; ++j) {
                const int8_t* fr[9]; for (int p2 = 0; p2 < 8; ++p2) fr[p2] = lf + ((size_t)(j - 1) * 8 + p2) * 1024; fr[8] = unit;
                yd[8] = rec[j];
                fr_t z; { const int rc = blk8_tile(fr, yd, 9, z); if (rc) return rc; }
                if (b == nb - 1) st[j] = z; else rec[j] = recode_signed(z);
            }
        }
        st[0] = s0;
        for (int r = half; r < k.rf; ++r) { const int rc = full(r, k.mds_frag); if (rc) return rc; }
        for (int j = 0; j < t; ++j) st4(states + 4 * (s * t + j), st[j]);
    }
    return 0;
}
size_t hc_blk8_table(void* h, int which, void* out, size_t cap) {
    HcParams* P = (HcParams*)h; const host::KernelConsts& k = P->kc;
    const void* src = which == 0 ? (const void*)k.blk8_efrag.data() : which == 1 ? (const void*)k.blk8_lfrag.data() : which == 3 ? (const void*)k.blk8_gfrag.data() : (const void*)k.gamma8_29.data();
    const size_t len = which == 0 ? k.blk8_efrag.size() : which == 1 ? k.blk8_lfrag.size() : which == 3 ? k.blk8_gfrag.size() : k.gamma8_29.size() * 4;
    if (out && len) memcpy(out, src, std::min(cap, len));
    return len;
}
int hc_blk8_finish_with_base(void* h, const int32_t* sums, const uint64_t* bases, size_t n, uint64_t* out) {
    HcParams* P = (HcParams*)h; if (P->kc.blk8_lfrag.empty()) return -3;
    const int8_t* unit = P->kc.blk8_lfrag.data() + P->kc.blk8_lfrag.size() - 1024;
    for (size_t s = 0; s < n; ++s) {
        const fr_t bd = recode_signed(ld4(bases + 4 * s)); int32_t U[32], S[32];
        if (blk8_tile_sums(&unit, &bd, 1, U)) return -1;
        for (int c = 0; c < 32; ++c) { const int64_t v = (int64_t)sums[32 * s + c] + U[c]; if (v >= (1 << 24) || v <= -(1 << 24)) return -1; S[c] = (int32_t)v; }
        st4(out + 4 * s, blk8_finish_sums(S));
    }
    return 0;
}
int hc_permute_kernel_form(void* h, uint64_t* states, size_t n) {
    HcParams* P = (HcParams*)h; int t = P->dev.t; std::vector<fr_t> st(t);
    for (size_t i = 0; i < n; ++i) { for (int j = 0; j < t; ++j) st[j] = ld4(states + 4 * (i * t + j)); ArrayState s{st.data()}; permute_core(s, P->dev, false); for (int j = 0; j < t; ++j) st4(states + 4 * (i * t + j), st[j]); }
    return 0;
}
int hc_permute_chain_model(void* h, uint64_t* states, size_t n) {
    HcParams* P = (HcParams*)h; const int t = P->ref.t, half = P->ref.rf / 2; if (!P->dev.chain_a) return -1;
    std::vector<fr_t> st(t), o(t);
    auto dense = [&](const std::vector<fr_t>& M) { for (int i = 0; i < t; ++i) { fr_t acc = host::h_zero(); for (int j = 0; j < t; ++j) acc = host::h_add(acc, host::h_mul(M[(size_t)i * t + j], st[j])); o[i] = acc; } st = o; };
    for (size_t i = 0; i < n; ++i) {
        for (int j = 0; j < t; ++j) st[j] = ld4(states + 4 * (i * t + j));
        for (int r = 0; r < half; ++r) { for (int j = 0; j < t; ++j) st[j] = fr_pow5<PallasFr>(host::h_add(st[j], P->ref.rc_full[(size_t)r * t + j])); dense(r == half - 1 ? P->kc.mds_pre : P->kc.mds); }
        chain_partial_model(st.data(), P->dev);
        for (int r = half; r < P->ref.rf; ++r) { for (int j = 0; j < t; ++j) st[j] = fr_pow5<PallasFr>(host::h_add(st[j], P->ref.rc_full[(size_t)r * t + j])); dense(P->kc.mds); }
        for (int j = 0; j < t; ++j) st4(states + 4 * (i * t + j), st[j]);
    }
    return 0;
}
int hc_row_consts(uint32_t* out14) { const RowConstsHost K = row_consts_host(); for (int i = 0; i < 9; ++i) out14[i] = K.ni[i]; for (int i = 0; i < 5; ++i) out14[9 + i] = K.t[i]; return 0; }
size_t hc_chain_table(void* h, int which, uint32_t* out, size_t cap) {
    HcParams* P = (HcParams*)h; const std::vector<uint32_t>& v = which == 0 ? P->kc.chain_a : which == 1 ? P->kc.chain_g : P->kc.chain_w;
    if (out) for (size_t i = 0; i < v.size() && i < cap; ++i) out[i] = v[i];
    return v.size();
}
int hc_permute_dense(void* h, uint64_t* states, size_t n) {
    HcParams* P = (HcParams*)h; int t = P->ref.t; std::vector<fr_t> st(t);
    for (size_t i = 0; i < n; ++i) { for (int j = 0; j < t; ++j) st[j] = ld4(states + 4 * (i * t + j)); host::permute_dense(st.data(), P->ref); for (int j = 0; j < t; ++j) st4(states + 4 * (i * t + j), st[j]); }
    return 0;
}
}
static void leaf_init(fr_t init[17]) {
    const fr_t AB = host::h_tag("FSv1-ABSORB-BYTES"), CH = host::h_tag("FSv1-CHALLENGE");
    for (int j = 0; j < 17; ++j) init[j] = host::h_zero();
    init[0] = AB; init[1] = host::h_words("FRI/leaf/poseidon")[0]; init[2] = AB; init[3] = host::h_words("FRI/leaf")[0];
    init[6] = CH; init[7] = AB; init[8] = host::h_words("leaf")[0]; init[16] = host::h_tag("FSv1-TRANSCRIPT-INIT");
}
extern "C" {
int hc_leaf_pair(void* tparams, const uint64_t* f, const uint64_t* f_next, size_t n, size_t m, uint64_t* hout) {
    HcParams* P = (HcParams*)tparams;
    fr_t init[17]; leaf_init(init);
    std::vector<fr_t> fv(n), nv(f_next ? (n + m - 1) / m : 0);
    for (size_t i = 0; i < fv.size(); ++i) fv[i] = ld4(f + 4 * i);
    for (size_t i = 0; i < nv.size(); ++i) nv[i] = ld4(f_next + 4 * i);
    const LeafStream L{init, fv.data(), f_next ? nv.data() : nullptr, m, n};
    fr_t st[17];
    for (size_t i = 0; i < n; ++i) { ArrayState s{st}; st4(hout + 4 * i, leaf_pair_body(s, P->dev, L, i)); }
    return 0;
}
int hc_hash_ds_level(void* params, int mode, size_t arity, uint32_t level, uint64_t pos0, uint64_t label, const uint64_t* in0, const uint64_t* in1, size_t n_in, uint64_t* out) {
    HcParams* P = (HcParams*)params;
    std::vector<fr_t> a(n_in), b(in1 ? n_in : 0), st(P->dev.t);
    for (size_t i = 0; i < n_in; ++i) { a[i] = ld4(in0 + 4 * i); if (in1) b[i] = ld4(in1 + 4 * i); }
    const DsStream D = DsStream::make(mode, arity, level, pos0, label, a.data(), in1 ? b.data() : nullptr, n_in);
    for (size_t k = 0; k < D.n_out; ++k) { ArrayState s{st.data()}; st4(out + 4 * k, hash_ds_body(s, P->dev, D, k)); }
    return 0;
}
int hc_tr_hash(void* tparams, const char* tag, const uint64_t* fields, size_t k, size_t n, uint64_t* out) {
    HcParams* P = (HcParams*)tparams;
    std::vector<fr_t> fr; const int np = host::tr_hash_frame(tag, fr);
    std::vector<fr_t> fl(n * k); for (size_t i = 0; i < n * k; ++i) fl[i] = ld4(fields + 4 * i);
    const TrStream T = TrStream::equal(fr.data(), np, (int)fr.size() - np, fl.data(), k, n, host::h_tag("FSv1-TRANSCRIPT-INIT"));
    fr_t st[17];
    for (size_t i = 0; i < n; ++i) { ArrayState s{st}; st4(out + 4 * i, tr_hash_body(s, P->dev, T, i)); }
    return 0;
}
int hc_tr_frame_dims(const char* tag, int* np, int* ns) { std::vector<fr_t> fr; *np = host::tr_hash_frame(tag, fr); *ns = (int)fr.size() - *np; return 0; }
int hc_tr_hash_many(void* tparams, size_t n, const char* const* tags, const uint64_t* const* fields, const size_t* k, uint64_t* out, size_t* launch_order) {
    HcParams* P = (HcParams*)tparams;
    std::vector<std::vector<fr_t>> frames(n), fl(n); std::vector<TrFrameRef> fr(n); std::vector<const fr_t*> fp(n, nullptr);
    for (size_t i = 0; i < n; ++i) {
        const int np = host::tr_hash_frame(tags[i], frames[i]); fr[i] = TrFrameRef{frames[i].data(), np, (int)frames[i].size() - np};
        if (!k[i]) continue;
        if (!fields || !fields[i]) return -1;
        fl[i].resize(k[i]); for (size_t q = 0; q < k[i]; ++q) fl[i][q] = ld4(fields[i] + 4 * q);
        fp[i] = fl[i].data();
    }
    const std::vector<TrStream::Item> items = tr_ragged_items(fr.data(), fp.data(), k, n);
    const TrStream T = tr_ragged_stream(items.data(), n, host::h_tag("FSv1-TRANSCRIPT-INIT"));
    fr_t st[17];
    for (size_t j = 0; j < n; ++j) {
        ArrayState s{st}; size_t slot = n; const fr_t d = tr_hash_body<true>(s, P->dev, T, j, &slot);
        if (slot >= n) return -2;
        st4(out + 4 * slot, d); if (launch_order) launch_order[j] = slot;
    }
    return 0;
}
size_t hc_mixed_prove_groups(size_t B, const size_t* n0, const size_t* schedule, const size_t* sched_off, const size_t* r, size_t* group_of, size_t* order) {
    const std::vector<std::vector<size_t>> G = mixed_prove_groups(B, n0, schedule, sched_off, r);
    size_t pos = 0;
    for (size_t g = 0; g < G.size(); ++g) for (size_t i : G[g]) { group_of[i] = g; order[pos++] = i; }
    return G.size();
}
int hc_hash_stream(void* params, int mode, const uint64_t* a, size_t na, const uint64_t* b, size_t nb, const uint64_t* tag, size_t n, uint64_t* out) {
    HcParams* P = (HcParams*)params;
    std::vector<fr_t> av(n * na), bv(n * nb), st(P->dev.t);
    for (size_t i = 0; i < n * na; ++i) av[i] = ld4(a + 4 * i); for (size_t i = 0; i < n * nb; ++i) bv[i] = ld4(b + 4 * i);
    for (size_t k = 0; k < n; ++k) { ArrayState s{st.data()}; st4(out + 4 * k, hash_stream_body(s, P->dev, mode, av.data(), na, bv.data(), nb, tag ? ld4(tag) : host::h_zero(), k)); }
    return 0;
}

struct HcHasher : TrHasher {
    void* tp; explicit HcHasher(void* p) : tp(p) {}
    int32_t hash(const char* tag, const fr_t* fields, size_t k, size_t n, fr_t* out) override {
        std::vector<uint64_t> in(4 * k * n), o(4 * n);
        for (size_t i = 0; i < k * n; ++i) st4(in.data() + 4 * i, fields[i]);
        int rc = hc_tr_hash(tp, tag, in.data(), k, n, o.data()); if (rc) return rc;
        for (size_t i = 0; i < n; ++i) out[i] = ld4(o.data() + 4 * i);
        return 0;
    }
};
struct HcPlan { FriPlan plan; void* tp; };
void* hc_fri_plan_create(void* tparams, const uint64_t* roots, size_t n0, const size_t* schedule, size_t L, size_t r) {
    std::vector<fr_t> rt(L + 1); for (size_t l = 0; l <= L; ++l) rt[l] = ld4(roots + 4 * l);
    HcPlan* P = new HcPlan(); P->tp = tparams; P->plan.r = r; std::string err;
    if (!P->plan.shape.make(n0, schedule, L, rt.data(), err)) { delete P; return nullptr; }
    HcHasher H(tparams); if (fri_plan_make(P->plan, H)) { delete P; return nullptr; }
    return P;
}
size_t hc_fri_plan_num_requests(void* p) { return ((HcPlan*)p)->plan.req.size(); }
int hc_fri_plan_requests(void* p, uint32_t* kind, uint32_t* which, uint32_t* level, uint64_t* index) {
    auto& rq = ((HcPlan*)p)->plan.req;
    for (size_t i = 0; i < rq.size(); ++i) { kind[i] = rq[i].kind; which[i] = rq[i].which; level[i] = rq[i].level; index[i] = rq[i].index; }
    return 0;
}
size_t hc_fri_plan_assemble(void* p, const uint64_t* values, size_t n_values, uint8_t* buf, size_t cap, size_t* est) {
    HcPlan* P = (HcPlan*)p; if (n_values != P->plan.req.size()) return 0;
    std::vector<fr_t> v(n_values); for (size_t i = 0; i < n_values; ++i) v[i] = ld4(values + 4 * i);
    ReplaySource src(v.data(), v.size()); HcHasher H(P->tp); std::vector<uint8_t> b; size_t e = 0;
    if (assemble_proof(P->plan.shape, P->plan.r, H, src, b, e) || src.pos != v.size()) return 0;
    if (est) *est = e;
    if (buf && cap >= b.size()) memcpy(buf, b.data(), b.size());
    return b.size();
}
void hc_fri_plan_free(void* p) { delete (HcPlan*)p; }

struct HcParamCache {
    std::map<int, HcParams*> mp;
    ~HcParamCache() { for (auto& kv : mp) delete kv.second; }
    HcParams* params(size_t arity) { int t = host::width_for_arity(arity); auto it = mp.find(t); if (it != mp.end()) return it->second; HcParams* P = new HcParams(); P->ref = host::consts_for_width(t); bind(P); mp[t] = P; return P; }
};
static HcParamCache& hc_param_cache() { static HcParamCache c; return c; }
static void run_plan_host(VerifyBatchPlan V, const HcParams* tparams, int32_t* accepted) {
    { std::vector<fr_t> dev = hc_fr_block(V.pool.size()); std::copy(V.pool.begin(), V.pool.begin() + V.n_known, dev.begin()); V.pool.swap(dev); }
    if (V.nl) {
        fr_t init[17]; leaf_init(init);
        const LeafStream LS{init, V.pool.data() + V.leaf_f0, V.pool.data() + V.leaf_f0 + V.nl, 1, V.nl};
        fr_t st[17]; for (size_t j = 0; j < V.nl; ++j) { ArrayState s{st}; V.pool[V.leaf_out0 + j] = leaf_pair_body(s, tparams->dev, LS, j); }
    }
    for (const VerifyBatchPlan::Group& G : V.groups) {
        HcParams* P = hc_param_cache().params((size_t)G.t - 1); std::vector<fr_t> st(P->dev.t);
        const DsGatherStream D{V.hdr.data() + 4 * G.job0, V.off.data() + G.job0, V.idx.data(), V.pool.data(), G.n, G.max_children};
        for (size_t k = 0; k < D.n_out; ++k) { ArrayState s{st.data()}; V.pool[G.out0 + k] = hash_ds_body(s, P->dev, D, k); }
    }
    for (size_t b = 0; b < V.batch; ++b) {
        int32_t acc = V.flag[b];
        for (uint32_t j = V.chk_off[b]; j < V.chk_off[b + 1]; ++j) acc &= fr_eq(V.pool[V.chk[2 * j]], V.pool[V.chk[2 * j + 1]]) ? 1 : 0;
        accepted[b] = acc;
    }
}
int hc_deep_fri_verify_batch(void* tparams, size_t batch, const uint8_t* const* proofs, const size_t* lens, const size_t* schedule, size_t L, size_t r, int32_t* accepted) {
    VerifyBatchPlanner pl; for (size_t b = 0; b < batch; ++b) pl.add(proofs[b], lens[b], schedule, L, r);
    if (!pl.fits_u32()) return -1;
    VerifyBatchPlan V; pl.finish(V);
    run_plan_host(std::move(V), (const HcParams*)tparams, accepted);
    return 0;
}
int hc_deep_fri_verify(void* tparams, const uint8_t* bytes, size_t len, const size_t* schedule, size_t L, size_t r) {
    int32_t acc = 0; const int rc = hc_deep_fri_verify_batch(tparams, 1, &bytes, &len, schedule, L, r, &acc);
    return rc ? rc : acc;
}
size_t hc_verify_batch_groups(size_t batch, const uint8_t* const* proofs, const size_t* lens, const size_t* schedule, size_t L, size_t r, int32_t* t, uint32_t* depth, size_t* n, size_t cap) {
    VerifyBatchPlanner pl; for (size_t b = 0; b < batch; ++b) pl.add(proofs[b], lens[b], schedule, L, r);
    VerifyBatchPlan V; pl.finish(V);
    for (size_t g = 0; g < V.groups.size() && g < cap; ++g) { t[g] = V.groups[g].t; depth[g] = V.groups[g].depth; n[g] = V.groups[g].n; }
    return V.groups.size();
}
int hc_merkle_verify(void* tparams, int pairs, size_t cfg_arity, uint64_t label, const uint64_t* root, const size_t* idx, size_t k, const uint64_t* vals, const uint64_t* cp, const uint8_t* proof, size_t len) {
    (void)tparams;
    const uint64_t none[4] = {0, 0, 0, 0};
    MerkleVerifyPlanner pl; pl.add(cfg_arity, label, root, idx, k, vals, pairs ? (cp ? cp : none) : nullptr, proof, len);
    if (!pl.fits_u32()) return -1;
    VerifyBatchPlan V; pl.finish(V);
    int32_t acc = 0; run_plan_host(std::move(V), nullptr, &acc);
    return acc;
}

}

struct ScHostExec {
    HcParams* cp; HcParams* tp; std::vector<std::vector<uint64_t>> mem;
    int32_t alloc(size_t bytes, void** out) { mem.push_back(hc_block(bytes)); *out = mem.back().data(); return 0; }
    int32_t upload(void* dst, const void* src, size_t bytes) { memcpy(dst, src, bytes); return 0; }
    int32_t download(void* dst, const void* src, size_t bytes) { memcpy(dst, src, bytes); return 0; }
    int32_t ds_level(const DsBatchStream& D, fr_t* out) {
        std::vector<fr_t> st(cp->dev.t);
        for (size_t k = 0; k < D.n_out; ++k) { ArrayState s{st.data()}; out[k] = hash_ds_body(s, cp->dev, D, k); }
        return 0;
    }
    int32_t coeffs(const fr_t* const* ptrs, const fr_t* layers, size_t len, size_t B, fr_t* c01, fr_t* claim) {
        for (size_t b = 0; b < B; ++b) {
            const fr_t* l = ptrs ? ptrs[b] : layers + b * len; fr_t c0 = fr_zero<PF>(), c1 = fr_zero<PF>();
            for (size_t j = 0; j < len / 2; ++j) { c0 = fr_add<PF>(c0, l[2 * j]); c1 = fr_add<PF>(c1, fr_sub<PF>(l[2 * j + 1], l[2 * j])); }
            c01[2 * b] = c0; c01[2 * b + 1] = c1; if (claim) claim[b] = fr_add<PF>(fr_add<PF>(c0, c0), c1);
        }
        return 0;
    }
    int32_t fold(const fr_t* const* ptrs, const fr_t* layers, size_t len, size_t B, const fr_t* r, fr_t* next) {
        for (size_t b = 0; b < B; ++b) {
            const fr_t* l = ptrs ? ptrs[b] : layers + b * len;
            for (size_t j = 0; j < len / 2; ++j) next[b * (len / 2) + j] = fr_add<PF>(l[2 * j], fr_mul<PF>(r[b], fr_sub<PF>(l[2 * j + 1], l[2 * j])));
        }
        return 0;
    }
    int32_t transcript(const TrBatchStream& T) { fr_t st[17]; for (size_t a = 0; a < T.n_active; ++a) { ArrayState s{st}; tr_batch_body(s, tp->dev, T, a); } return 0; }
    int32_t gather(const fr_t* const* addr, size_t n, fr_t* out) { for (size_t j = 0; j < n; ++j) out[j] = *addr[j]; return 0; }
};
extern "C" {
int hc_hash_ds_batch_level(void* params, size_t arity, uint32_t level, uint64_t pos0, const uint64_t* labels, const uint64_t* in, size_t n_in, size_t trees, int by_ptrs, uint64_t* out) {
    HcParams* P = (HcParams*)params;
    std::vector<fr_t> a(n_in * trees), st(P->dev.t); for (size_t i = 0; i < a.size(); ++i) a[i] = ld4(in + 4 * i);
    std::vector<const fr_t*> ptrs(trees); for (size_t b = 0; b < trees; ++b) ptrs[b] = a.data() + b * n_in;
    const DsBatchStream D = DsBatchStream::make(arity, level, pos0, labels, by_ptrs ? ptrs.data() : nullptr, by_ptrs ? nullptr : a.data(), n_in, trees);
    for (size_t k = 0; k < D.n_out; ++k) { ArrayState s{st.data()}; st4(out + 4 * k, hash_ds_body(s, P->dev, D, k)); }
    return 0;
}
int hc_tr_batch(void* tparams, uint64_t* state, uint32_t* pos, size_t n_inst, const uint32_t* inst, size_t inst0, size_t n_active, size_t nseg, const uint32_t* el_off,
                const uint32_t* idx, const uint64_t* pool0, size_t n0, const uint64_t* pool1, size_t n1, int reset, int finish_last, uint64_t* out) {
    HcParams* P = (HcParams*)tparams;
    std::vector<fr_t> st(17 * n_inst), p0(n0), p1(n1), o(n_active * nseg, host::h_zero());
    for (size_t i = 0; i < st.size(); ++i) st[i] = ld4(state + 4 * i);
    for (size_t i = 0; i < n0; ++i) p0[i] = ld4(pool0 + 4 * i); for (size_t i = 0; i < n1; ++i) p1[i] = ld4(pool1 + 4 * i);
    TrBatchStream T; T.state = st.data(); T.pos = pos; T.inst = inst; T.inst0 = inst0; T.n_active = n_active; T.nseg = nseg; T.el_off = el_off; T.idx = idx;
    T.pool0 = p0.data(); T.pool1 = p1.data(); T.out = o.data(); T.init_cap = host::h_tag("FSv1-TRANSCRIPT-INIT"); T.reset = reset; T.finish_last = finish_last;
    fr_t s17[17]; for (size_t a = 0; a < n_active; ++a) { ArrayState s{s17}; tr_batch_body(s, P->dev, T, a); }
    for (size_t i = 0; i < st.size(); ++i) st4(state + 4 * i, st[i]);
    for (size_t i = 0; i < o.size(); ++i) st4(out + 4 * i, o[i]);
    return 0;
}
size_t hc_sumcheck_prove_batch(void* tparams, void* cparams, int mf, size_t B, const uint64_t* const* witnesses, size_t k, const uint64_t* labels, size_t q,
                               uint8_t* buf, size_t cap, size_t* lens) {
    const size_t n = (size_t)1 << k;
    std::vector<std::vector<fr_t>> w(B, std::vector<fr_t>(n)); std::vector<const fr_t*> wp(B);
    for (size_t b = 0; b < B; ++b) { for (size_t i = 0; i < n; ++i) w[b][i] = ld4(witnesses[b] + 4 * i); wp[b] = w[b].data(); }
    ScHostExec X{(HcParams*)cparams, (HcParams*)tparams, {}};
    ScBatch<ScHostExec> S(X, B, wp.data(), k, labels);
    std::vector<std::vector<uint8_t>> pr;
    if (mf ? S.prove_mf(q, pr) : S.prove_plain(pr)) return 0;
    size_t tot = 0; for (size_t b = 0; b < B; ++b) { lens[b] = pr[b].size(); tot += pr[b].size(); }
    if (buf && cap >= tot) { size_t o = 0; for (auto& p : pr) { memcpy(buf + o, p.data(), p.size()); o += p.size(); } }
    return tot;
}
}

static int sc_verify_plan(int mf, size_t batch, const uint8_t* const* proofs, const size_t* lens, const uint64_t* labels, ScVerifyPlan& V) {
    bool fits = false;
    if (sc_verify_plan_some(mf, 0, batch, proofs, lens, labels, (size_t)-1, V, fits) != batch || !fits) return -1;
    return 0;
}
extern "C" {
int hc_sc_decode_fr(const uint8_t* blob, size_t len, size_t off, uint64_t* out4) {
    if (off + 32 > len) return -1;
    std::vector<uint32_t> w((len + 3) / 4 + 2, 0u); memcpy(w.data(), blob, len);
    fr_t x; const bool ok = sc_decode_fr(w.data(), (uint32_t)off, 0u, x); st4(out4, x); return ok ? 1 : 0;
}
int hc_sumcheck_verify_batch(void* tparams, void* cparams, int mf, size_t batch, const uint8_t* const* proofs, const size_t* lens, const uint64_t* labels, int32_t* accepted) {
    ScVerifyPlan V; if (sc_verify_plan(mf, batch, proofs, lens, labels, V)) return -1;
    HcParams *tp = (HcParams*)tparams, *cp = (HcParams*)cparams;
    std::vector<fr_t> pool = hc_fr_block(std::max<size_t>(V.pool_slots, 1));
    for (size_t j = 0; j < V.n_dec; ++j) if (!sc_decode_fr(V.blob.data(), V.dec_off[j], V.dec_proof[j], pool[j])) V.flag[V.dec_proof[j] & ~kScClaim] = 0;
    std::vector<fr_t> state = hc_fr_block(17 * std::max<size_t>(V.n_inst, 1)); std::vector<uint32_t> pos(std::max<size_t>(V.n_inst, 1), 0x01010101u * (uint32_t)g_alloc_fill);
    for (const ScVerifyPlan::Stream& S : V.tr) {
        TrBatchStream T; T.state = state.data(); T.pos = pos.data(); T.inst = nullptr; T.inst0 = S.inst0; T.n_active = S.n; T.nseg = S.nseg; T.el_off = V.tr_off.data() + S.seg0;
        T.idx = V.tr_idx.data(); T.pool0 = pool.data(); T.pool1 = V.consts.data(); T.out = pool.data() + V.n_dec + S.seg0; T.init_cap = host::h_tag("FSv1-TRANSCRIPT-INIT"); T.reset = 1; T.finish_last = 1;
        fr_t st[17]; for (size_t a = 0; a < S.n; ++a) { ArrayState s{st}; tr_batch_body(s, tp->dev, T, a); }
    }
    for (const VerifyBatchPlan::Group& G : V.ds.groups) {
        std::vector<fr_t> st(cp->dev.t);
        const DsGatherStream D{V.ds.hdr.data() + 4 * G.job0, V.ds.off.data() + G.job0, V.ds.idx.data(), pool.data(), G.n, G.max_children};
        for (size_t k = 0; k < D.n_out; ++k) { ArrayState s{st.data()}; pool[G.out0 + k] = hash_ds_body(s, cp->dev, D, k); }
    }
    for (size_t j = 0; j < V.n_rec(); ++j) {
        const uint32_t* r = V.rec.data() + 8 * j;
        if (!(mf ? sc_check_mf(pool.data(), r) : sc_check_plain(pool.data(), r))) V.flag[mf ? r[1] : r[0]] = 0;
    }
    for (size_t b = 0; b < batch; ++b) accepted[b] = V.flag[b];
    return 0;
}
size_t hc_sumcheck_verify_batch_steps(int mf, size_t batch, const uint8_t* const* proofs, const size_t* lens, const uint64_t* labels, int32_t* kind, size_t* count, size_t cap) {
    ScVerifyPlan V; if (sc_verify_plan(mf, batch, proofs, lens, labels, V)) return 0;
    const auto st = V.steps();
    for (size_t i = 0; i < st.size() && i < cap; ++i) { kind[i] = st[i].first; count[i] = st[i].second; }
    return st.size();
}
}

struct FriHostExec {
    HcParams* tp; std::vector<std::vector<uint64_t>> mem;
    HcParamCache& mp;
    explicit FriHostExec(HcParams* t) : tp(t), mp(hc_param_cache()) {}
    int32_t alloc(size_t bytes, void** out) { mem.push_back(hc_block(bytes)); *out = mem.back().data(); return 0; }
    int32_t upload(void* dst, const void* src, size_t bytes) { memcpy(dst, src, bytes); return 0; }
    int32_t zpows(const fr_t& z, size_t m, fr_t* zp) { fr_t acc = fr_one<PF>(); for (size_t t = 0; t < m; ++t) { zp[t] = acc; acc = fr_mul<PF>(acc, z); } return 0; }
    int32_t fold(const fr_t* f, size_t n, const fr_t* zp, size_t m, fr_t* out) {
        for (size_t b = 0; b < n / m; ++b) { fr_t acc = fr_zero<PF>(); for (size_t t = 0; t < m; ++t) acc = fr_add<PF>(acc, fr_mul<PF>(f[b * m + t], zp[t])); out[b] = acc; }
        return 0;
    }
    int32_t leaf_pairs(const fr_t* f, const fr_t* f_next, size_t n, size_t m, fr_t* h) {
        fr_t init[17]; leaf_init(init); const LeafStream LS{init, f, f_next, m, n};
        fr_t st[17]; for (size_t i = 0; i < n; ++i) { ArrayState s{st}; h[i] = leaf_pair_body(s, tp->dev, LS, i); }
        return 0;
    }
    template <class DS> int32_t ds(size_t arity, const DS& D, fr_t* out) {
        HcParams* P = mp.params(arity); std::vector<fr_t> st(P->dev.t);
        for (size_t k = 0; k < D.n_out; ++k) { ArrayState s{st.data()}; out[k] = hash_ds_body(s, P->dev, D, k); }
        return 0;
    }
    int32_t pair_level(size_t arity, const DsBatchPairStream& D, fr_t* out) { return ds(arity, D, out); }
    int32_t ds_level(size_t arity, const DsBatchStream& D, fr_t* out) { return ds(arity, D, out); }
    int32_t fork() { return 0; }
    void side(bool) {}
    int32_t join() { return 0; }
};
extern "C" {
int hc_hash_ds_batch_pairs_level(void* params, size_t arity, const uint64_t* labels, const uint64_t* f, const uint64_t* cp, size_t n, size_t cp_div, size_t trees, uint64_t* out) {
    HcParams* P = (HcParams*)params;
    if (!cp_div || n % cp_div) return -1;
    std::vector<fr_t> a(n * trees), b(cp ? n / cp_div * trees : 0), st(P->dev.t);
    for (size_t i = 0; i < a.size(); ++i) a[i] = ld4(f + 4 * i);
    for (size_t i = 0; i < b.size(); ++i) b[i] = ld4(cp + 4 * i);
    const DsBatchPairStream D = DsBatchPairStream::make(arity, labels, a.data(), cp ? b.data() : nullptr, n, cp_div, trees);
    for (size_t k = 0; k < D.n_out; ++k) { ArrayState s{st.data()}; st4(out + 4 * k, hash_ds_body(s, P->dev, D, k)); }
    return 0;
}
int hc_fri_commit_batch(void* tparams, size_t B, const uint64_t* const* f0, size_t n0, const size_t* schedule, size_t L, uint64_t seed_z, uint64_t* roots) {
    FriHostExec X((HcParams*)tparams); FriBatchCommit<FriHostExec> C(X);
    std::string err; if (int rc = C.shape(B, n0, schedule, L, err)) return rc;
    HcHasher H(tparams); std::vector<fr_t> z(L);
    for (size_t l = 0; l < L; ++l) {
        const fr_t in[3] = {host::h_u64(seed_z), host::h_u64(l), host::h_u64(C.n[l])}; fr_t fused; if (H.hash("FRI/z/l", in, 3, 1, &fused)) return -3;
        z[l] = fri_z_from_fused(fused, seed_z, l, C.n[l]);
    }
    if (int rc = C.init(z.data())) return rc;
    for (size_t b = 0; b < B; ++b) for (size_t i = 0; i < n0; ++i) C.f[0][b * n0 + i] = ld4(f0[b] + 4 * i);
    if (int rc = C.run()) return rc;
    for (size_t b = 0; b < B; ++b) for (size_t l = 0; l <= L; ++l) st4(roots + 4 * (b * (L + 1) + l), C.roots[l * B + b]);
    return 0;
}
}

extern "C" {
size_t hc_ntt_batch_passes(size_t batch, int log_out, size_t max_elems, size_t* out, size_t cap) {
    const std::vector<size_t> p = ntt_batch_passes(batch, log_out, max_elems);
    for (size_t i = 0; i < p.size() && i < cap; ++i) out[i] = p[i];
    return p.size();
}
int hc_ntt_batch_ranges_overlap(const uint64_t* starts, size_t batch, size_t bytes) {
    std::vector<const void*> p(batch); for (size_t i = 0; i < batch; ++i) p[i] = (const void*)(uintptr_t)starts[i];
    return ntt_batch_ranges_overlap(p.data(), batch, bytes) ? 1 : 0;
}
}

template <int C>
static void mle_pass_host(bool contig, size_t B, const fr_t* const* ptrs, const fr_t* layers, uint64_t len, int t, const fr_t* r, size_t k, size_t j0, fr_t* next) {
    const int x = t - C; const uint64_t blocks = ((len >> C) + 255) / 256;
    for (size_t b = 0; b < B; ++b) {
        const fr_t* layer = ptrs ? ptrs[b] : layers + b * len; const fr_t* rr = r + b * k + j0; fr_t* dst = next + b * (len >> t);
        for (uint64_t blk = 0; blk < blocks; ++blk) {
            fr_t v[256], u[256]; MleLane L[256]; bool live[256];
            for (int tid = 0; tid < 256; ++tid) {
                L[tid] = mle_lane(blk * 256 + tid, t, C, contig); live[tid] = L[tid].first < len;
                v[tid] = live[tid] ? mle_fold_local<C>(layer + L[tid].first, L[tid].stride, rr + L[tid].local0) : fr_zero<PF>();
            }
            for (int s = 0; s < 6 && s < x; ++s) {
                for (int tid = 0; tid < 256; ++tid) u[tid] = mle_fold1(v[tid], v[tid ^ (1 << s)], rr[L[tid].cross0 + s]);
                std::copy(u, u + 256, v);
            }
            if (x <= 6) { for (int tid = 0; tid < 256; ++tid) if (live[tid] && (tid & ((1 << x) - 1)) == 0) dst[L[tid].tile] = v[tid]; continue; }
            const fr_t w[4] = {v[0], v[64], v[128], v[192]};
            for (int tid = 0; tid < (4 >> (x - 6)); ++tid) {
                const uint64_t tile = (blk << (kMleLogThreads - x)) + tid;
                if ((tile << t) < len) dst[tile] = mle_fold_waves(w, x, tid, rr[L[tid].cross0 + 6], x == 8 ? rr[L[tid].cross0 + 7] : fr_zero<PF>());
            }
        }
    }
}
extern "C" {
int hc_mle_evaluate_batch(size_t B, const uint64_t* const* tables, size_t k, const uint64_t* r, int log_tile, int contig, uint64_t* out, size_t* passes) {
    const int T = log_tile < 0 ? kMleDefaultLogTile : log_tile;
    if (T < kMleMinLogTile || T > kMleMaxLogTile || k > 40) return -1;
    const bool cg = (contig < 0 ? kMleDefaultContig : contig) != 0;
    const std::vector<int> rounds = mle_pass_rounds(k, T);
    if (passes) *passes = rounds.size();
    std::vector<std::vector<fr_t>> tab(B, std::vector<fr_t>((size_t)1 << k)); std::vector<const fr_t*> ptrs(B); std::vector<fr_t> rv(B * k);
    for (size_t b = 0; b < B; ++b) { for (size_t i = 0; i < tab[b].size(); ++i) tab[b][i] = ld4(tables[b] + 4 * i); ptrs[b] = tab[b].data(); }
    for (size_t i = 0; i < rv.size(); ++i) rv[i] = ld4(r + 4 * i);
    if (k == 0) { for (size_t b = 0; b < B; ++b) st4(out + 4 * b, tab[b][0]); return 0; }
    std::vector<fr_t> cur, nxt; size_t j0 = 0;
    for (size_t i = 0; i < rounds.size(); ++i) {
        const int t = rounds[i]; const uint64_t len = (uint64_t)1 << (k - j0);
        nxt = hc_fr_block(B * (len >> t));
        switch (mle_local_rounds(t)) {
            case 0: mle_pass_host<0>(cg, B, i ? nullptr : ptrs.data(), cur.data(), len, t, rv.data(), k, j0, nxt.data()); break;
            case 1: mle_pass_host<1>(cg, B, i ? nullptr : ptrs.data(), cur.data(), len, t, rv.data(), k, j0, nxt.data()); break;
            case 2: mle_pass_host<2>(cg, B, i ? nullptr : ptrs.data(), cur.data(), len, t, rv.data(), k, j0, nxt.data()); break;
            case 3: mle_pass_host<3>(cg, B, i ? nullptr : ptrs.data(), cur.data(), len, t, rv.data(), k, j0, nxt.data()); break;
            case 4: mle_pass_host<4>(cg, B, i ? nullptr : ptrs.data(), cur.data(), len, t, rv.data(), k, j0, nxt.data()); break;
            default: return -1;
        }
        cur.swap(nxt); j0 += (size_t)t;
    }
    for (size_t b = 0; b < B; ++b) st4(out + 4 * b, cur[b]);
    return 0;
}
}
extern "C" int hc_mle_default_log_tile() { return kMleDefaultLogTile; }

struct LagHostExec {
    std::vector<std::vector<uint64_t>> mem; std::vector<fr_t> lo, hi;
    int32_t alloc(size_t bytes, void** out) { mem.push_back(hc_block(bytes)); *out = mem.back().data(); return 0; }
    template <class T> int32_t put(const std::vector<T>& h, T** out) {
        void* p = nullptr; alloc(std::max<size_t>(h.size(), 1) * sizeof(T), &p);
        if (!h.empty()) memcpy(p, h.data(), h.size() * sizeof(T));
        *out = (T*)p; return 0;
    }
    int32_t pow_table(const fr_t& omega, size_t n, LagPow* out) {
        int bits, lo_bits, hi_bits; lag_pow_split(n, &bits, &lo_bits, &hi_bits);
        lo.assign((size_t)1 << lo_bits, fr_one<PF>()); hi.assign((size_t)1 << hi_bits, fr_one<PF>());
        for (size_t i = 1; i < lo.size(); ++i) lo[i] = fr_mul<PF>(lo[i - 1], omega);
        const fr_t step = fr_pow_u64<PF>(omega, (uint64_t)1 << lo_bits);
        for (size_t i = 1; i < hi.size(); ++i) hi[i] = fr_mul<PF>(hi[i - 1], step);
        *out = LagPow{lo.data(), hi.data(), lo_bits}; return 0;
    }
    int32_t gather(const fr_t* const* cols, size_t ncols, const uint64_t* j, const uint64_t* slot, size_t cnt, fr_t* out) {
        for (size_t q = 0; q < cnt; ++q) for (size_t c = 0; c < ncols; ++c) out[slot[q] * ncols + c] = cols[c][j[q]];
        return 0;
    }
    int32_t partials(const fr_t* const* cols, size_t ncols, size_t n, const LagPow& wp, const fr_t& w_step, const fr_t& w_step_inv, const fr_t* zs, size_t npts, unsigned groups, unsigned grid, fr_t* part) {
        const uint32_t T = grid * 256, n32 = (uint32_t)n;
        std::vector<fr_t> Wv(256 * kLagK), w(256), run(256), lane(256);
        auto W = [&](int t) -> fr_t (&)[kLagK] { return *reinterpret_cast<fr_t (*)[kLagK]>(&Wv[(size_t)t * kLagK]); };
        for (unsigned g = 0; g < groups; ++g) for (unsigned blk = 0; blk < grid; ++blk) {
            for (int t = 0; t < 256; ++t) { const uint32_t tid = blk * 256 + t; w[t] = tid < n32 ? lag_pow(wp, tid) : fr_one<PF>(); }
            for (size_t p = g; p < npts; p += groups) {
                const fr_t z = zs[p];
                for (int t = 0; t < 256; ++t) run[t] = lag_prefix(z, w[t], w_step, blk * 256 + (uint32_t)t, T, n32, W(t));
                fr_t tot[4], P = fr_one<PF>();
                for (int v = 0; v < 4; ++v) { tot[v] = fr_one<PF>(); for (int l = 0; l < 64; ++l) tot[v] = fr_mul<PF>(tot[v], run[64 * v + l]); P = fr_mul<PF>(P, tot[v]); }
                const fr_t Pinv = fr_inv<PF>(P);
                for (int t = 0; t < 256; ++t) {
                    const int v = t >> 6, l = t & 63; fr_t before = fr_one<PF>(), after = fr_one<PF>();
                    for (int q = 0; q < l; ++q) before = fr_mul<PF>(before, run[64 * v + q]);
                    for (int q = l + 1; q < 64; ++q) after = fr_mul<PF>(after, run[64 * v + q]);
                    lag_peel(z, w[t], w_step_inv, blk * 256 + (uint32_t)t, T, n32, lag_lane_inverse(Pinv, tot, v, fr_mul<PF>(before, after)), W(t));
                }
                for (size_t c = 0; c < ncols; ++c) {
                    for (int t = 0; t < 256; ++t) lane[t] = lag_lane_dot<kLagWideAcc>(cols[c], blk * 256 + (uint32_t)t, T, n32, W(t));
                    fr_t w4[4];
                    for (int v = 0; v < 4; ++v) { w4[v] = fr_zero<PF>(); for (int l = 0; l < 64; ++l) w4[v] = fr_add<PF>(w4[v], lane[64 * v + l]); }
                    part[(p * ncols + c) * grid + blk] = lag_sum4(w4);
                }
            }
        }
        return 0;
    }
    int32_t finish(const fr_t* part, unsigned grid, const fr_t* scale, const uint64_t* slot, size_t npts, size_t ncols, fr_t* out) {
        for (size_t b = 0; b < npts * ncols; ++b) {
            const size_t p = b / ncols, c = b % ncols; fr_t lane[256];
            for (int t = 0; t < 256; ++t) { lane[t] = fr_zero<PF>(); for (size_t i = (size_t)t; i < grid; i += 256) lane[t] = fr_add<PF>(lane[t], part[b * grid + i]); }
            fr_t w4[4];
            for (int w = 0; w < 4; ++w) { w4[w] = fr_zero<PF>(); for (int l = 0; l < 64; ++l) w4[w] = fr_add<PF>(w4[w], lane[64 * w + l]); }
            out[slot[p] * ncols + c] = fr_mul<PF>(lag_sum4(w4), scale[p]);
        }
        return 0;
    }
};
extern "C" {
int hc_lagrange_eval_batch(size_t ncols, const uint64_t* const* cols, size_t n, const uint64_t* omega, size_t npoints, const uint64_t* z, size_t max_partials, uint64_t* out, size_t* passes) {
    if (passes) *passes = 0;
    if (!ncols || !npoints) return 0;
    if (!n || (n & (n - 1)) || n > ((size_t)1 << kLagMaxLogN)) return -1;
    int lg = 0; while (((size_t)1 << lg) < n) ++lg;
    const fr_t w = omega ? ld4(omega) : fr_root_of_unity<PF>((unsigned)lg);
    if (lag_check_domain(n, w)) return -1;
    std::vector<std::vector<fr_t>> col(ncols, std::vector<fr_t>(n)); std::vector<const fr_t*> ptrs(ncols); std::vector<fr_t> zs(npoints);
    for (size_t c = 0; c < ncols; ++c) {
        size_t first = c; for (size_t q = 0; q < c; ++q) if (cols[q] == cols[c]) { first = q; break; }
        if (first == c) for (size_t i = 0; i < n; ++i) col[c][i] = ld4(cols[c] + 4 * i);
        ptrs[c] = col[first].data();
    }
    for (size_t p = 0; p < npoints; ++p) zs[p] = ld4(z + 4 * p);
    std::vector<fr_t> o = hc_fr_block(npoints * ncols);
    LagHostExec X;
    if (lagrange_eval_batch(X, ncols, ptrs.data(), n, w, npoints, zs.data(), max_partials ? max_partials : kLagDefaultMaxPartials, o.data(), passes)) return -1;
    for (size_t i = 0; i < o.size(); ++i) st4(out + 4 * i, o[i]);
    return 0;
}
}

struct MerkleHostExec {
    HcParams* p; std::vector<std::vector<uint64_t>> mem; std::vector<uint64_t> labels; std::vector<const fr_t*> lv, cpv;
    int32_t level_block(size_t n_fr, fr_t** out) {
        mem.emplace_back(4 * n_fr + 1, g_alloc_fill ? 0x0101010101010101ull * (uint64_t)g_alloc_fill : 0xA5A5A5A5A5A5A5A5ull); *out = (fr_t*)mem.back().data(); return 0;
    }
    int32_t tables(const uint64_t* l, const fr_t* const* leaves, const fr_t* const* cp, size_t B, const uint64_t** lx, const fr_t* const** vx, const fr_t* const** cx) {
        labels.assign(l, l + B); lv.assign(leaves, leaves + B); if (cp) cpv.assign(cp, cp + B);
        *lx = labels.data(); *vx = lv.data(); *cx = cp ? cpv.data() : nullptr; return 0;
    }
    int32_t copy_rows(const fr_t* const* src, size_t n, size_t B, fr_t* dst) { for (size_t b = 0; b < B; ++b) for (size_t i = 0; i < n; ++i) dst[b * n + i] = src[b][i]; return 0; }
    template <class DS> int32_t ds(const DS& D, fr_t* out) {
        std::vector<fr_t> st(p->dev.t);
        for (size_t k = 0; k < D.n_out; ++k) { ArrayState s{st.data()}; out[k] = hash_ds_body(s, p->dev, D, k); }
        return 0;
    }
    int32_t pair_level(const DsBatchPairPtrStream& D, fr_t* out) { return ds(D, out); }
    int32_t ds_level(const DsBatchStream& D, fr_t* out) { return ds(D, out); }
};
struct MerkleOpenHostExec { int32_t gather(const MerkleGatherList& G, fr_t* out) { for (size_t i = 0; i < G.size(); ++i) out[G.row_of(i)] = G.base[G.src[i]][G.index[i]]; return 0; } };
static std::vector<size_t> total_lens(const std::vector<size_t>& lens, size_t B) { std::vector<size_t> o(lens.size() + 1, 0); for (size_t v = 0; v < lens.size(); ++v) o[v + 1] = o[v] + B * lens[v]; return o; }
extern "C" {
int hc_merkle_build_batch(void* params, size_t arity, size_t B, const uint64_t* labels, const uint64_t* const* leaves, size_t n, int pairs, const uint64_t* const* cp,
                          uint64_t* out, size_t cap_fr, size_t* lens_out) {
    HcParams* P = (HcParams*)params;
    if (!B || !n || !arity || host::width_for_arity(arity) != P->dev.t || (arity == 1 && n > 1) || (pairs && !cp)) return -1;
    std::vector<std::vector<fr_t>> col(B, std::vector<fr_t>(n)), cc(B); std::vector<const fr_t*> lp(B), cpp(B, nullptr);
    for (size_t b = 0; b < B; ++b) {
        for (size_t i = 0; i < n; ++i) col[b][i] = ld4(leaves[b] + 4 * i);
        lp[b] = col[b].data();
        if (pairs && cp[b]) { cc[b].resize(n); for (size_t i = 0; i < n; ++i) cc[b][i] = ld4(cp[b] + 4 * i); cpp[b] = cc[b].data(); }
    }
    MerkleHostExec X{P, {}, {}, {}, {}}; std::vector<size_t> lens; std::vector<fr_t*> base;
    if (merkle_build_batch(X, arity, B, labels, lp.data(), n, pairs, pairs ? cpp.data() : nullptr, lens, base)) return -1;
    const std::vector<size_t> at = total_lens(lens, B);
    if (lens.size() > 64 || at.back() > cap_fr) return -1;
    for (size_t v = 0; v < lens.size(); ++v) { lens_out[v] = lens[v]; for (size_t i = 0; i < B * lens[v]; ++i) st4(out + 4 * (at[v] + i), base[v][i]); }
    return (int)lens.size();
}
long hc_merkle_open_batch(size_t B, const size_t* arity, const size_t* nlev, const uint64_t* const* levels, const size_t* lens, const size_t* idx, const size_t* idx_off,
                          uint8_t* buf, size_t cap, size_t* out_lens) {
    std::vector<std::vector<std::vector<fr_t>>> lv(B); std::vector<std::vector<const fr_t*>> lp(B); std::vector<std::vector<size_t>> ll(B); std::vector<MerkleTreeView> views(B);
    for (size_t b = 0, q = 0; b < B; ++b) {
        for (size_t v = 0; v < nlev[b]; ++v, ++q) {
            lv[b].emplace_back(lens[q]); for (size_t i = 0; i < lens[q]; ++i) lv[b][v][i] = ld4(levels[q] + 4 * i);
            ll[b].push_back(lens[q]);
        }
        for (auto& l : lv[b]) lp[b].push_back(l.data());
        views[b] = MerkleTreeView{arity[b], &ll[b], lp[b].data()};
    }
    MerkleOpenHostExec X; std::vector<std::vector<uint8_t>> pr;
    if (merkle_open_batch(X, views.data(), B, idx, idx_off, pr)) return -1;
    size_t tot = 0; for (size_t b = 0; b < B; ++b) { out_lens[b] = pr[b].size(); tot += pr[b].size(); }
    if (buf && cap >= tot) { size_t o = 0; for (auto& p : pr) { memcpy(buf + o, p.data(), p.size()); o += p.size(); } }
    return (long)tot;
}
int hc_merkle_verify_batch(size_t cfg_arity, size_t batch, const uint64_t* labels, const uint64_t* roots, const size_t* indices, const size_t* idx_off, const uint64_t* values,
                           const uint8_t* const* proofs, const size_t* lens, size_t max_slots, int32_t* accepted) {
    if (host::width_for_arity(cfg_arity) < 0 || cfg_arity == 0) return -1;
    auto run = [](const VerifyBatchPlan& V, int32_t* acc) { run_plan_host(V, nullptr, acc); return 0; };
    return merkle_verify_batch(run, cfg_arity, batch, labels, roots, indices, idx_off, values, proofs, lens, max_slots ? max_slots : (size_t)1 << 25, accepted);
}
}
```

### stark_mlwe_amd/csrc/mfma_digits.hpp

```cpp
#pragma once
#include "fr.hpp"
#include "fr29.hpp"

namespace stark {

FR_HD fr_t recode_signed(const fr_t& x) {
    fr_t y; uint64_t c = 0;
#pragma unroll
    for (int i = 0; i < 8; ++i) { const uint64_t t = (uint64_t)x.v[i] + 0x80808080u + c; y.v[i] = (uint32_t)t ^ 0x80808080u; c = t >> 32; }
    return y;
}
template <class V> FR_HD void mfma_fold_rows(int64_t* col, const V& lo, const V& hi) {
#pragma unroll
    for (int q = 0; q < 4; ++q)
#pragma unroll
        for (int hh = 0; hh < 2; ++hh)
#pragma unroll
            for (int p = 0; p < 2; ++p) {
                const V& a = hh ? hi : lo;
                const int64_t pair = (int64_t)a[4 * q + 2 * p] + (int64_t)a[4 * q + 2 * p + 1] * 256;
                const int c = 8 * q + 4 * hh + 2 * p, k = (8 * c) / 29, sh = 8 * c - 29 * k;
                col[k] += pair * ((int64_t)1 << sh);
            }
}
FR_HD fr_t mfma_finish_cols(int64_t* col) {
    typedef PallasFr PF;
    static_assert(fr_p29<PF>(4) < (1u << 10) && fr_p29<PF>(5) == 0 && fr_p29<PF>(6) == 0 && fr_p29<PF>(7) == 0 && fr_p29<PF>(8) == (1u << 22), "r = 2^254 + t with t below 2^126");
    uint32_t l[9];
#pragma unroll
    for (int k = 0; k < 8; ++k) { col[k + 1] += col[k] >> 29; l[k] = (uint32_t)col[k] & FR_M29; }
    const int64_t top = col[8];
    const int32_t q1 = (int32_t)(top >> 22) - 1;
    l[8] = ((uint32_t)top & ((1u << 22) - 1)) + (1u << 22);
    int64_t carry = 0;
#pragma unroll
    for (int i = 0; i < 5; ++i) { const int64_t d = (int64_t)l[i] - (int64_t)q1 * (int64_t)fr_p29<PF>(i) + carry; l[i] = (uint32_t)d & FR_M29; carry = d >> 29; }
    int32_t c32 = (int32_t)carry;
#pragma unroll
    for (int i = 5; i < 9; ++i) { const int32_t d = (int32_t)l[i] + c32; if (i < 8) { l[i] = (uint32_t)d & FR_M29; c32 = d >> 29; } else l[8] = (uint32_t)d; }
    fr_t z = fr29_pack_reduce<PF>(l);
    fr_cond_sub<PF>(z.v, 0u);
    return z;
}

}
```

### stark_mlwe_amd/csrc/poseidon_pair.hpp

```cpp
#pragma once
#include "fr.hpp"
#include "dev_common.hpp"
#include "poseidon_params.hpp"
#include "poseidon_dev.hpp"
#include "poseidon_streams.hpp"

#if defined(__HIPCC__)
namespace stark {

template <int T> struct PairCfg {
#ifndef STARK_NXD17
#define STARK_NXD17 5
#endif
    static constexpr int NXD = T == 17 ? STARK_NXD17 : 2;
#ifndef STARK_NXU17
#define STARK_NXU17 8
#endif
    static constexpr int NXU = T == 17 ? STARK_NXU17 : (T - 1) / 2;
    static constexpr int NX = (T - 1) / 2;
    static constexpr int EXTRA = 3;
    __host__ __device__ static constexpr int xslot(int p) { return p == 0 ? 0 : T + (p - 1); }
    __host__ __device__ static constexpr int dslot(int q) { return 1 + (q % NXD); }
    __host__ __device__ static constexpr size_t lds_bytes() { return (size_t)(T + EXTRA) * 2 * 64 * 16; }
};
static inline size_t pair_lds_bytes(int t) { return t == 17 ? PairCfg<17>::lds_bytes() : PairCfg<9>::lds_bytes(); }

struct PairState {
    uint4* st;
    int lane; bool isY;
    __device__ __forceinline__ fr_t ld(int j) const {
        uint4 lo = st[(2 * j) * 64 + lane], hi = st[(2 * j + 1) * 64 + lane];
        fr_t x; x.v[0] = lo.x; x.v[1] = lo.y; x.v[2] = lo.z; x.v[3] = lo.w; x.v[4] = hi.x; x.v[5] = hi.y; x.v[6] = hi.z; x.v[7] = hi.w; return x;
    }
    __device__ __forceinline__ void sto(int j, const fr_t& x) const {
        st[(2 * j) * 64 + lane] = make_uint4(x.v[0], x.v[1], x.v[2], x.v[3]);
        st[(2 * j + 1) * 64 + lane] = make_uint4(x.v[4], x.v[5], x.v[6], x.v[7]);
    }
};

template <int T>
__device__ __forceinline__ void pair_apply_lu(const PairState& s, const uint32_t* lu) {
    const int yo = s.isY ? 1 : 0;
#pragma unroll 1
    for (int k = 0; 2 * k < T; ++k) {
        const int i = 2 * k + yo; const bool have = i < T;
        fr_t res;
        if (have) { DotAcc w; w.init(); _Pragma("unroll 1") for (int j = i; j < T; ++j) w.mac(c29(lu, i * T + j), s.ld(j)); res = w.finish(); }
        __syncthreads();
        if (have) s.sto(i, res);
    }
    __syncthreads();
#pragma unroll 1
    for (int k = 0; T - 1 - 2 * k >= 1; ++k) {
        const int i = T - 1 - 2 * k - yo; const bool have = i >= 1;
        fr_t res;
        if (have) { DotAcc w; w.init(); _Pragma("unroll 1") for (int j = 0; j < i; ++j) w.mac(c29(lu, i * T + j), s.ld(j)); res = fr_add<PF>(s.ld(i), w.finish()); }
        __syncthreads();
        if (have) s.sto(i, res);
    }
    __syncthreads();
}
__device__ __forceinline__ fr_t recode_signed(const fr_t& x) {
    fr_t y; uint64_t c = 0;
#pragma unroll
    for (int i = 0; i < 8; ++i) { const uint64_t t = (uint64_t)x.v[i] + 0x80808080u + c; y.v[i] = (uint32_t)t ^ 0x80808080u; c = t >> 32; }
    return y;
}
template <int T, bool RECODE = false>
__device__ __forceinline__ void pair_sbox_full(const PairState& s, const fr_t* rc) {
    const int j0 = s.isY ? PairCfg<T>::NX : 0, j1 = s.isY ? T : PairCfg<T>::NX;
    for (int j = j0; j < j1; ++j) { const fr_t x = fr_pow5_r29<PF>(fr_add<PF>(s.ld(j), rc[j])); s.sto(j, RECODE ? recode_signed(x) : x); }
    __syncthreads();
}

typedef int mfma_v4i __attribute__((ext_vector_type(4)));
typedef int mfma_v16i __attribute__((ext_vector_type(16)));
__device__ __forceinline__ void mfma_fold_rows(int64_t* col, const mfma_v16i& lo, const mfma_v16i& hi) {
#pragma unroll
    for (int q = 0; q < 4; ++q)
#pragma unroll
        for (int hh = 0; hh < 2; ++hh)
#pragma unroll
            for (int p = 0; p < 2; ++p) {
                const mfma_v16i& a = hh ? hi : lo;
                const int64_t pair = (int64_t)a[4 * q + 2 * p] + (int64_t)a[4 * q + 2 * p + 1] * 256;
                const int c = 8 * q + 4 * hh + 2 * p, k = (8 * c) / 29, sh = 8 * c - 29 * k;
                col[k] += pair * ((int64_t)1 << sh);
            }
}
__device__ __forceinline__ fr_t mfma_finish_cols(int64_t* col) {
    uint32_t l[9];
#pragma unroll
    for (int k = 0; k < 8; ++k) { col[k + 1] += col[k] >> 29; l[k] = (uint32_t)col[k] & FR_M29; }
    const int64_t top = col[8];
    const int32_t q1 = (int32_t)(top >> 22) - 1;
    l[8] = ((uint32_t)top & ((1u << 22) - 1)) + (1u << 22);
    int64_t carry = 0;
#pragma unroll
    for (int i = 0; i < 5; ++i) { const int64_t d = (int64_t)l[i] - (int64_t)q1 * (int64_t)fr_p29<PF>(i) + carry; l[i] = (uint32_t)d & FR_M29; carry = d >> 29; }
    int32_t c32 = (int32_t)carry;
#pragma unroll
    for (int i = 5; i < 9; ++i) { const int32_t d = (int32_t)l[i] + c32; if (i < 8) { l[i] = (uint32_t)d & FR_M29; c32 = d >> 29; } else l[8] = (uint32_t)d; }
    fr_t z = fr29_pack_reduce<PF>(l);
    fr_cond_sub<PF>(z.v, 0u);
    return z;
}
__device__ __forceinline__ void pair_apply_mds_mfma(const PairState& s, const void* frag) {
    constexpr int T = 17;
    static_assert(fr_p29<PF>(4) < (1u << 10) && fr_p29<PF>(5) == 0 && fr_p29<PF>(6) == 0 && fr_p29<PF>(7) == 0 && fr_p29<PF>(8) == (1u << 22), "r = 2^254 + t with t below 2^126");
    const int lane = s.lane, h = lane >> 5;
    mfma_v4i b[T][2];
#pragma unroll
    for (int e = 0; e < T; ++e)
#pragma unroll
        for (int ct = 0; ct < 2; ++ct) { const uint4 u = s.st[(2 * e + h) * 64 + 32 * ct + (lane & 31)]; b[e][ct] = mfma_v4i{(int)u.x, (int)u.y, (int)u.z, (int)u.w}; }
    __syncthreads();
    const mfma_v4i* A = reinterpret_cast<const mfma_v4i*>(frag) + lane;
#pragma unroll 1
    for (int i = s.isY ? 1 : 0; i < T; i += 2) {
        mfma_v16i acc[2];
#pragma unroll
        for (int ct = 0; ct < 2; ++ct)
#pragma unroll
            for (int r = 0; r < 16; ++r) acc[ct][r] = 0;
        const mfma_v4i* Ai = A + (size_t)i * T * 64;
#pragma unroll
        for (int e = 0; e < T; ++e) {
            const mfma_v4i a = Ai[(size_t)e * 64];
#pragma unroll
            for (int ct = 0; ct < 2; ++ct) acc[ct] = __builtin_amdgcn_mfma_i32_32x32x32_i8(a, b[e][ct], acc[ct], 0, 0, 0);
        }
        mfma_v16i lo, hi;
#pragma unroll
        for (int r = 0; r < 16; ++r) {
            const auto sw = __builtin_amdgcn_permlane32_swap((unsigned)acc[0][r], (unsigned)acc[1][r], false, false);
            lo[r] = (int)sw[0]; hi[r] = (int)sw[1];
        }
        int64_t col[9];
#pragma unroll
        for (int k = 0; k < 9; ++k) col[k] = 0;
        mfma_fold_rows(col, lo, hi);
        s.sto(i, mfma_finish_cols(col));
    }
    __syncthreads();
}

struct Blk8Tabs {
    const mfma_v4i* efrag;
    const mfma_v4i* lfrag;
    const mfma_v4i* unit;
    const mfma_v4i* gfrag;
    const uint32_t* a29;
    const fr_t* rc;
};
struct Blk8Cfg {
    static constexpr int NLX = 8;
    __host__ __device__ static constexpr int ymail(int q) { return 17 + (q & 1); }
    __host__ __device__ static constexpr int hmail(int q) { return (q & 1) ? 19 : 0; }
};
__device__ __forceinline__ fr_t mfma_post(const mfma_v16i (&acc)[2]) {
    mfma_v16i lo, hi;
#pragma unroll
    for (int r = 0; r < 16; ++r) {
        const auto sw = __builtin_amdgcn_permlane32_swap((unsigned)acc[0][r], (unsigned)acc[1][r], false, false);
        lo[r] = (int)sw[0]; hi[r] = (int)sw[1];
    }
    int64_t col[9];
#pragma unroll
    for (int k = 0; k < 9; ++k) col[k] = 0;
    mfma_fold_rows(col, lo, hi);
    return mfma_finish_cols(col);
}
__device__ __forceinline__ void blk8_load_frags16(mfma_v4i (&a)[16], const mfma_v4i* A, int lane) {
#pragma unroll
    for (int e = 0; e < 16; ++e) a[e] = (A + (size_t)e * 64)[lane];
}
__device__ __forceinline__ mfma_v4i blk8_b_of_slot(const PairState& s, int j, int ct) {
    const uint4 u = s.st[(2 * j + (s.lane >> 5)) * 64 + 32 * ct + (s.lane & 31)];
    return mfma_v4i{(int)u.x, (int)u.y, (int)u.z, (int)u.w};
}
template <int Q>
__device__ __forceinline__ void blk8_round_x(const PairState& s, const Blk8Tabs& Tb, fr_t& s0, mfma_v4i (&b)[8][2]) {
    __builtin_amdgcn_sched_barrier(0);
    const fr_t y = fr_pow5_r29<PF>(fr_add<PF>(s0, Tb.rc[Q]));
    fr_wide29 acc; fr_wide29_zero(acc);
    fr_wide29_mac(acc, c29(Tb.a29, (size_t)Q * (2 * 17 - 1)), fr29_unpack(y));
    const fr_t part = fr_wide29_reduce<PF>(acc);
    s.sto(Blk8Cfg::ymail(Q), recode_signed(y));
    __syncthreads();
    s0 = fr_add<PF>(part, s.ld(Blk8Cfg::hmail(Q)));
    b[Q][0] = blk8_b_of_slot(s, Blk8Cfg::ymail(Q), 0); b[Q][1] = blk8_b_of_slot(s, Blk8Cfg::ymail(Q), 1);
}
template <int Q>
__device__ __forceinline__ void blk8_round_y(const PairState& s, const Blk8Tabs& Tb, mfma_v4i (&b)[8][2], mfma_v4i (&a)[16], mfma_v4i (&g)[7]) {
    __builtin_amdgcn_sched_barrier(0);
    const int lane = s.lane;
    mfma_v16i acc[2];
#pragma unroll
    for (int ct = 0; ct < 2; ++ct)
#pragma unroll
        for (int r = 0; r < 16; ++r) acc[ct][r] = 0;
#pragma unroll
    for (int e = 0; e < 16; ++e)
#pragma unroll
        for (int ct = 0; ct < 2; ++ct) acc[ct] = __builtin_amdgcn_mfma_i32_32x32x32_i8(a[e], blk8_b_of_slot(s, e + 1, ct), acc[ct], 0, 0, 0);
    if constexpr (Q > 0) {
#pragma unroll
        for (int p = 0; p < Q; ++p)
#pragma unroll
            for (int ct = 0; ct < 2; ++ct) acc[ct] = __builtin_amdgcn_mfma_i32_32x32x32_i8(g[p], b[p][ct], acc[ct], 0, 0, 0);
    }
    if constexpr (Q < 7) {
        blk8_load_frags16(a, Tb.efrag + (size_t)(Q + 1) * 16 * 64, lane);
#pragma unroll
        for (int p = 0; p <= Q; ++p) g[p] = (Tb.gfrag + (size_t)((Q + 1) * Q / 2 + p) * 64)[lane];
    }
    s.sto(Blk8Cfg::hmail(Q), mfma_post(acc));
    __syncthreads();
    b[Q][0] = blk8_b_of_slot(s, Blk8Cfg::ymail(Q), 0); b[Q][1] = blk8_b_of_slot(s, Blk8Cfg::ymail(Q), 1);
}
template <int NLX>
__device__ __forceinline__ void blk8_lane_rows(const PairState& s, const Blk8Tabs& Tb, const mfma_v4i (&b)[8][2], bool last) {
    static_assert(NLX >= 1 && NLX <= 15, "shares");
    const int lane = s.lane;
    const int j0 = s.isY ? NLX + 1 : 1, j1 = s.isY ? 16 : NLX;
    const mfma_v4i aunit = Tb.unit[lane];
    mfma_v4i a[8];
#pragma unroll
    for (int p = 0; p < 8; ++p) a[p] = (Tb.lfrag + ((size_t)(j0 - 1) * 8 + p) * 64)[lane];
#pragma unroll 1
    for (int j = j0; j <= j1; ++j) {
        mfma_v16i acc[2];
#pragma unroll
        for (int ct = 0; ct < 2; ++ct)
#pragma unroll
            for (int r = 0; r < 16; ++r) acc[ct][r] = 0;
#pragma unroll
        for (int p = 0; p < 8; ++p)
#pragma unroll
            for (int ct = 0; ct < 2; ++ct) acc[ct] = __builtin_amdgcn_mfma_i32_32x32x32_i8(a[p], b[p][ct], acc[ct], 0, 0, 0);
#pragma unroll
        for (int ct = 0; ct < 2; ++ct) acc[ct] = __builtin_amdgcn_mfma_i32_32x32x32_i8(aunit, blk8_b_of_slot(s, j, ct), acc[ct], 0, 0, 0);
        const int jn = j < j1 ? j + 1 : j1;
#pragma unroll
        for (int p = 0; p < 8; ++p) a[p] = (Tb.lfrag + ((size_t)(jn - 1) * 8 + p) * 64)[lane];
        const fr_t z = mfma_post(acc);
        s.sto(j, last ? z : recode_signed(z));
    }
    __syncthreads();
}
template <int NLX>
__device__ __forceinline__ void pair_block8(const PairState& s, const Blk8Tabs& Tb, fr_t& s0, bool last) {
    mfma_v4i b[8][2];
    if (!s.isY) {
        blk8_round_x<0>(s, Tb, s0, b); blk8_round_x<1>(s, Tb, s0, b); blk8_round_x<2>(s, Tb, s0, b); blk8_round_x<3>(s, Tb, s0, b);
        blk8_round_x<4>(s, Tb, s0, b); blk8_round_x<5>(s, Tb, s0, b); blk8_round_x<6>(s, Tb, s0, b); blk8_round_x<7>(s, Tb, s0, b);
    } else {
        mfma_v4i a[16], g[7];
        blk8_load_frags16(a, Tb.efrag, s.lane);
        blk8_round_y<0>(s, Tb, b, a, g); blk8_round_y<1>(s, Tb, b, a, g); blk8_round_y<2>(s, Tb, b, a, g); blk8_round_y<3>(s, Tb, b, a, g);
        blk8_round_y<4>(s, Tb, b, a, g); blk8_round_y<5>(s, Tb, b, a, g); blk8_round_y<6>(s, Tb, b, a, g); blk8_round_y<7>(s, Tb, b, a, g);
    }
    __builtin_amdgcn_sched_barrier(0);
    blk8_lane_rows<NLX>(s, Tb, b, last);
}

template <int T>
__device__ __forceinline__ fr_t pair_lane_update(const uint32_t* sp, int j, const fr_t& base, const fr29_t& x0, const fr29_t& x1, const fr29_t& x2, const fr29_t& x3) {
    constexpr int W = 2 * T - 1;
    fr_wide29 u; fr_wide29_zero(u);
    fr_wide29_mac(u, c29(sp, 0 * W + T - 1 + j), x0); fr_wide29_mac(u, c29(sp, 1 * W + T - 1 + j), x1);
    fr_wide29_mac(u, c29(sp, 2 * W + T - 1 + j), x2); fr_wide29_mac(u, c29(sp, 3 * W + T - 1 + j), x3);
    return fr_add<PF>(base, fr_wide29_reduce_lazy<PF>(u));
}

template <int T, bool BLK8 = false>
__device__ __forceinline__ fr_t pair_permute(const PairState& s, const PoseidonDev& P, bool only0, int r_begin = 0) {
    static_assert(!BLK8 || T == 17, "8-round blocks exist for t = 17");
    typedef PairCfg<T> Cfg;
    constexpr int NXD = Cfg::NXD, NXU = Cfg::NXU, W = 2 * T - 1;
    const int half = P.rf / 2;
    for (int r = r_begin; r < half; ++r) {
        if constexpr (T == 17) { pair_sbox_full<T, true>(s, P.rc_full + r * T); pair_apply_mds_mfma(s, (r == half - 1) ? P.mds_pre_frag : P.mds_frag); }
        else { pair_sbox_full<T>(s, P.rc_full + r * T); pair_apply_lu<T>(s, (r == half - 1) ? P.lu_pre29 : P.lu29); }
    }
    fr_t s0 = fr_zero<PF>();
    if (!s.isY) s0 = s.ld(0);
    if constexpr (BLK8) {
        for (int j = s.isY ? 9 : 1; j <= (s.isY ? 16 : 8); ++j) s.sto(j, recode_signed(s.ld(j)));
        __syncthreads();
        const int nb = P.rp / 8;
#pragma unroll 1
        for (int b = 0; b < nb; ++b) {
            const Blk8Tabs Tb{reinterpret_cast<const mfma_v4i*>(P.blk8_efrag) + (size_t)b * 8 * 16 * 64, reinterpret_cast<const mfma_v4i*>(P.blk8_lfrag) + (size_t)b * 16 * 8 * 64,
                              reinterpret_cast<const mfma_v4i*>(P.blk8_unit_frag), reinterpret_cast<const mfma_v4i*>(P.blk8_gfrag) + (size_t)b * 28 * 64,
                              c29(P.sparse29, (size_t)(8 * b) * W), P.rc_partial + 8 * b};
            pair_block8<Blk8Cfg::NLX>(s, Tb, s0, b == nb - 1);
        }
    } else
    for (int b = 0; b < P.rp / 4; ++b) {
        const uint32_t* sp = c29(P.sparse29, (size_t)(4 * b) * W);
        const uint32_t* g = c29(P.gamma29, (size_t)b * 6);
        if (!s.isY) {
            fr_t keep[NXD];
#pragma unroll
            for (int j = 0; j < NXD; ++j) keep[j] = s.ld(1 + j);
            __syncthreads();
#define STARK_PAIR_ROUND(q)                                                                           \
            {                                                                                         \
                __builtin_amdgcn_sched_barrier(0);                      \
                const fr_t xq = fr_pow5_r29<PF>(fr_add<PF>(s0, P.rc_partial[4 * b + q]));              \
                s.sto(Cfg::xslot(q), xq);                                                             \
                fr_wide29 acc; fr_wide29_zero(acc);                                                   \
                fr_wide29_mac(acc, c29(sp, q * W), fr29_unpack(xq));                                  \
                if (q > 0) fr_wide29_mac(acc, c29(g, q * (q - 1) / 2 + 0), fr29_unpack(s.ld(Cfg::xslot(0)))); \
                if (q > 1) fr_wide29_mac(acc, c29(g, q * (q - 1) / 2 + 1), fr29_unpack(s.ld(Cfg::xslot(1)))); \
                if (q > 2) fr_wide29_mac(acc, c29(g, q * (q - 1) / 2 + 2), fr29_unpack(s.ld(Cfg::xslot(2)))); \
                if (1 + q + NXD > fr29_max_terms<PF>()) fr_wide29_norm(acc);    \
                _Pragma("unroll") for (int j = 0; j < NXD; ++j) fr_wide29_mac(acc, c29(sp, q * W + 1 + j), fr29_unpack(keep[j])); \
                const fr_t part = fr_wide29_reduce<PF>(acc);                                          \
                __syncthreads();                                        \
                s0 = fr_add<PF>(part, s.ld(Cfg::dslot(q)));                                           \
            }
            STARK_PAIR_ROUND(0) STARK_PAIR_ROUND(1) STARK_PAIR_ROUND(2) STARK_PAIR_ROUND(3)
#undef STARK_PAIR_ROUND
            const fr29_t x0 = fr29_unpack(s.ld(Cfg::xslot(0))), x1 = fr29_unpack(s.ld(Cfg::xslot(1))), x2 = fr29_unpack(s.ld(Cfg::xslot(2))), x3 = fr29_unpack(s.ld(Cfg::xslot(3)));
#pragma unroll
            for (int j = 1; j <= NXD; ++j) { __builtin_amdgcn_sched_barrier(0); s.sto(j, pair_lane_update<T>(sp, j, keep[j - 1], x0, x1, x2, x3)); }
#pragma unroll 1
            for (int j = NXD + 1; j <= NXU; ++j) s.sto(j, pair_lane_update<T>(sp, j, s.ld(j), x0, x1, x2, x3));
        } else {
            __syncthreads();
            for (int q = 0; q < 4; ++q) {
                DotAcc acc; acc.init();
#pragma unroll 1
                for (int j = NXD + 1; j < T; ++j) acc.mac(c29(sp, q * W + j), s.ld(j));
                const fr_t dy = acc.finish();
                s.sto(Cfg::dslot(q), dy);
                __syncthreads();
            }
            const fr29_t x0 = fr29_unpack(s.ld(Cfg::xslot(0))), x1 = fr29_unpack(s.ld(Cfg::xslot(1))), x2 = fr29_unpack(s.ld(Cfg::xslot(2))), x3 = fr29_unpack(s.ld(Cfg::xslot(3)));
#pragma unroll 1
            for (int j = NXU + 1; j < T; ++j) s.sto(j, pair_lane_update<T>(sp, j, s.ld(j), x0, x1, x2, x3));
        }
        __syncthreads();
    }
    if (!s.isY) s.sto(0, s0);
    __syncthreads();
    for (int r = half; r < P.rf; ++r) {
        const bool squeeze = only0 && r == P.rf - 1;
        if constexpr (T == 17) { if (squeeze) pair_sbox_full<T>(s, P.rc_full + r * T); else pair_sbox_full<T, true>(s, P.rc_full + r * T); }
        else pair_sbox_full<T>(s, P.rc_full + r * T);
        if (squeeze) {
            const int j0 = s.isY ? Cfg::NX : 0, j1 = s.isY ? T : Cfg::NX;
            DotAcc acc; acc.init();
#pragma unroll 1
            for (int j = j0; j < j1; ++j) acc.mac(c29(P.row0_29, j), s.ld(j));
            s.sto(T + (s.isY ? 1 : 0), acc.finish());
            __syncthreads();
            fr_t out = fr_add<PF>(s.ld(T + 0), s.ld(T + 1));
            __syncthreads();
            return out;
        }
        if constexpr (T == 17) pair_apply_mds_mfma(s, P.mds_frag); else pair_apply_lu<T>(s, P.lu29);
    }
    return s.ld(0);
}

__device__ __forceinline__ PairState pair_setup(uint4* lds) {
    PairState s; s.st = lds; s.lane = threadIdx.x & 63;
    s.isY = __builtin_amdgcn_readfirstlane((int)(threadIdx.x >> 6)) != 0;
    return s;
}

template <bool BLK8>
__global__ void __launch_bounds__(128) __attribute__((amdgpu_waves_per_eu(2))) k_leaf_pair2(PoseidonDev P, const fr_t* __restrict__ leafc, const fr_t* __restrict__ f,
                                                    const fr_t* __restrict__ f_next, size_t n, size_t m, fr_t* __restrict__ h) {
    extern __shared__ uint4 lds[];
    PairState s = pair_setup(lds);
    const size_t i = (size_t)blockIdx.x * 64 + s.lane; const bool live = i < n; const size_t ii = live ? i : n - 1;
    const fr_t x4 = fr_pow5_r29<PF>(fr_add<PF>(ldg(f + ii), P.rc_full[4]));
    const fr_t x5 = fr_pow5_r29<PF>(fr_add<PF>(f_next ? ldg(f_next + ii / m) : fr_zero<PF>(), P.rc_full[5]));
    const int j0 = s.isY ? PairCfg<17>::NX : 0, j1 = s.isY ? 17 : PairCfg<17>::NX;
    const uint32_t* m45 = reinterpret_cast<const uint32_t*>(leafc + 51);
    const fr29_t x4u = fr29_unpack(x4), x5u = fr29_unpack(x5);
    for (int j = j0; j < j1; ++j) {
        fr_wide29 w; fr_wide29_zero(w);
        fr_wide29_mac(w, c29(m45, j), x4u); fr_wide29_mac(w, c29(m45, 17 + j), x5u);
        s.sto(j, fr_add<PF>(leafc[j], fr_wide29_reduce<PF>(w)));
    }
    __syncthreads();
    fr_t out = pair_permute<17, BLK8>(s, P, true, 1);
    if (live && !s.isY) stg(h + i, out);
}

template <int T, class DS, bool BLK8 = false>
__global__ void __launch_bounds__(128) __attribute__((amdgpu_waves_per_eu(2))) k_hash_ds2(PoseidonDev P, DS D, fr_t* __restrict__ out) {
    extern __shared__ uint4 lds[];
    constexpr int rate = T - 1;
    PairState s = pair_setup(lds);
    const size_t k0 = (size_t)blockIdx.x * 64 + s.lane; const bool live = k0 < D.n_out; const size_t k = live ? k0 : D.n_out - 1;
    const int o0 = s.isY ? PairCfg<T>::NX : 0, o1 = s.isY ? T : PairCfg<T>::NX;
    for (int j = o0; j < o1; ++j) s.sto(j, fr_zero<PF>());
    __syncthreads();
    const size_t total = D.total(k), nperm = (total + rate - 1) / rate;
    const size_t max_perm = (D.max_total() + rate - 1) / rate;
    const size_t skip = max_perm - nperm;
    size_t q = 0; fr_t res = fr_zero<PF>();
    for (size_t pidx = 0; pidx < max_perm; ++pidx) {
        if (pidx >= skip) {
            if (skip && pidx == skip) for (int j = o0; j < o1; ++j) s.sto(j, fr_zero<PF>());
            for (int cur = 0; cur < rate && q < total; ++cur, ++q) {
                if (cur < o0 || cur >= o1) continue;
                s.sto(cur, fr_add<PF>(s.ld(cur), D.elem(k, q)));
            }
        }
        __syncthreads();
        res = pair_permute<T, BLK8>(s, P, pidx + 1 == max_perm);
        __syncthreads();
    }
    if (live && !s.isY) stg(out + k0, res);
}

template <bool BLK8>
__global__ void __launch_bounds__(128) __attribute__((amdgpu_waves_per_eu(2))) k_node16_pair(PoseidonDev P, fr_t arity_f, fr_t level_f, fr_t label_f, uint64_t pos0,
                                                    const fr_t* __restrict__ in, size_t n_out, fr_t* __restrict__ out) {
    extern __shared__ uint4 lds[];
    PairState s = pair_setup(lds);
    const size_t k0 = (size_t)blockIdx.x * 64 + s.lane; const bool live = k0 < n_out; const size_t k = live ? k0 : n_out - 1;
    const fr_t* c = in + k * 16;
    static_assert(PairCfg<17>::NX == 8, "X fills elements 0..7");
    if (!s.isY) {
        s.sto(0, arity_f); s.sto(1, level_f); s.sto(2, fr_from_u64<PF>(pos0 + k)); s.sto(3, label_f);
#pragma unroll
        for (int j = 4; j < 8; ++j) s.sto(j, ldg(c + (j - 4)));
    } else {
#pragma unroll
        for (int j = 8; j < 16; ++j) s.sto(j, ldg(c + (j - 4)));
        s.sto(16, fr_zero<PF>());
    }
    __syncthreads();
    pair_permute<17, BLK8>(s, P, false);
    if (!s.isY) {
#pragma unroll
        for (int j = 0; j < 4; ++j) s.sto(j, fr_add<PF>(s.ld(j), ldg(c + 12 + j)));
        s.sto(4, fr_add<PF>(s.ld(4), fr_one<PF>()));
    }
    __syncthreads();
    const fr_t res = pair_permute<17, BLK8>(s, P, true);
    if (live && !s.isY) stg(out + k0, res);
}

}
#endif
```

### stark_mlwe_amd/csrc/poseidon_params.hpp

```cpp
#pragma once
#include "fr.hpp"
namespace stark {
struct PoseidonDev {
    int t, rf, rp;
    const fr_t* rc_full;
    const fr_t* rc_partial;
    const fr_t* lu;
    const fr_t* lu_pre;
    const fr_t* row0;
    const fr_t* sparse;
    const fr_t* mds;
    const fr_t* mds_pre;
    const fr_t* gamma;
    const uint32_t* lu29; const uint32_t* lu_pre29; const uint32_t* row0_29; const uint32_t* sparse29; const uint32_t* gamma29;
    const uint32_t* mds29; const uint32_t* mds_pre29;
    const void* mds_frag; const void* mds_pre_frag;
    const uint32_t* chain_a; const uint32_t* chain_g; const uint32_t* chain_w;
    const void* blk8_efrag; const void* blk8_lfrag; const void* blk8_unit_frag; const void* blk8_gfrag;
};

}
```

Measured before the change: 11.12 million trace rows/s.

## Fuse MFMA MDS output with next round's S-box using lazy radix-29 limbs

Adds a fused Poseidon full-round path for t=17 with the 8-round-block partial layer. Each MFMA MDS product now ends in unreduced radix-29 limbs, adds the next round's constant precomputed in radix-29 form, and applies x^5 right away. This skips the separate reduce, pack, store, sync and reload S-box pass between rounds, and it also fuses the hand-over from the partial block into the first second-half full round. The cost is more register pressure inside the MFMA loop and reliance on lazy-reduction bounds, which are checked only by the new host checks. The sponge kernel opts out of the fusion.

After: 11.34 million trace rows/s, median of 6. 1.02x the previous value.

```diff
diff --git a/stark_mlwe_amd/csrc/capi_core.hip b/stark_mlwe_amd/csrc/capi_core.hip
--- a/stark_mlwe_amd/csrc/capi_core.hip
+++ b/stark_mlwe_amd/csrc/capi_core.hip
@@ -99,7 +99,7 @@
     std::vector<fr_t> blob; auto put = [&](const std::vector<fr_t>& v) { size_t off = blob.size(); blob.insert(blob.end(), v.begin(), v.end()); return off; };
     size_t o_rcf = put(k.rc_full), o_rcp = put(k.rc_partial), o_lu = put(k.lu), o_pre = put(k.lu_pre), o_row0 = put(k.row0), o_sp = put(k.sparse), o_mds = put(k.mds), o_mpre = put(k.mds_pre), o_gam = put(k.gamma);
     const size_t o_29 = blob.size();
-    { std::vector<uint32_t> w29; for (auto* v : {&k.lu29, &k.lu_pre29, &k.row0_29, &k.sparse29, &k.gamma29, &k.mds29, &k.mds_pre29, &k.chain_a, &k.chain_g, &k.chain_w}) w29.insert(w29.end(), v->begin(), v->end());
+    { std::vector<uint32_t> w29; for (auto* v : {&k.lu29, &k.lu_pre29, &k.row0_29, &k.sparse29, &k.gamma29, &k.mds29, &k.mds_pre29, &k.chain_a, &k.chain_g, &k.chain_w, &k.rc_full29}) w29.insert(w29.end(), v->begin(), v->end());
       while (w29.size() % 8) w29.push_back(0);
       blob.resize(o_29 + w29.size() / 8); memcpy((void*)(blob.data() + o_29), w29.data(), w29.size() * 4); }
     const size_t o_frag = blob.size(), frag_elems = (k.mds_frag.size() + sizeof(fr_t) - 1) / sizeof(fr_t);
@@ -119,7 +119,8 @@
       P->dev.sparse29 = P->dev.row0_29 + k.row0_29.size(); P->dev.gamma29 = P->dev.sparse29 + k.sparse29.size();
       P->dev.mds29 = P->dev.gamma29 + k.gamma29.size(); P->dev.mds_pre29 = P->dev.mds29 + k.mds29.size();
       const uint32_t* ch = P->dev.mds_pre29 + k.mds_pre29.size();
-      P->dev.chain_a = k.chain_a.empty() ? nullptr : ch; P->dev.chain_g = k.chain_a.empty() ? nullptr : ch + k.chain_a.size(); P->dev.chain_w = k.chain_a.empty() ? nullptr : ch + k.chain_a.size() + k.chain_g.size(); }
+      P->dev.chain_a = k.chain_a.empty() ? nullptr : ch; P->dev.chain_g = k.chain_a.empty() ? nullptr : ch + k.chain_a.size(); P->dev.chain_w = k.chain_a.empty() ? nullptr : ch + k.chain_a.size() + k.chain_g.size();
+      P->dev.rc_full29 = ch + k.chain_a.size() + k.chain_g.size() + k.chain_w.size(); }
     P->dev.blk8_efrag = k.blk8_efrag.empty() ? nullptr : (const void*)(dev + o_b8); P->dev.blk8_lfrag = k.blk8_efrag.empty() ? nullptr : (const void*)(dev + o_b8 + ef_elems);
     P->dev.blk8_gfrag = k.blk8_gfrag.empty() ? nullptr : (const void*)(dev + o_b8 + ef_elems + lf_elems);
     P->dev.blk8_unit_frag = k.blk8_efrag.empty() ? nullptr : (const void*)((const int8_t*)P->dev.blk8_lfrag + k.blk8_lfrag.size() - 1024);
diff --git a/stark_mlwe_amd/csrc/host_util.hpp b/stark_mlwe_amd/csrc/host_util.hpp
--- a/stark_mlwe_amd/csrc/host_util.hpp
+++ b/stark_mlwe_amd/csrc/host_util.hpp
@@ -171,6 +171,7 @@
     std::vector<fr_t> gamma;
     std::vector<uint32_t> lu29, lu_pre29, row0_29, sparse29, gamma29;
     std::vector<uint32_t> mds29, mds_pre29;
+    std::vector<uint32_t> rc_full29;
     std::vector<int8_t> mds_frag, mds_pre_frag;
     std::vector<uint32_t> chain_a, chain_g, chain_w;
     std::vector<int8_t> blk8_efrag, blk8_lfrag, blk8_gfrag;
@@ -264,6 +265,8 @@
     k.lu29 = to_radix29(k.lu, upper); k.lu_pre29 = to_radix29(k.lu_pre, upper); k.row0_29 = to_radix29(k.row0, all);
     k.sparse29 = to_radix29(k.sparse, a_and_w); k.gamma29 = to_radix29(k.gamma, all);
     k.mds29 = to_radix29(k.mds, all); k.mds_pre29 = to_radix29(k.mds_pre, all);
+    k.rc_full29.resize(k.rc_full.size() * 9);
+    for (size_t i = 0; i < k.rc_full.size(); ++i) { const fr29_t u = fr29_unpack(k.rc_full[i]); for (int j = 0; j < 9; ++j) k.rc_full29[9 * i + j] = u.l[j]; }
     if (t == 17) { k.mds_frag = mfma_frags(k.mds, t); k.mds_pre_frag = mfma_frags(k.mds_pre, t); }
     if (t == 17 && c.rp % 8 == 0) {
         const int nb = c.rp / 8, w = 2 * t - 1;
diff --git a/stark_mlwe_amd/csrc/hostcheck.cpp b/stark_mlwe_amd/csrc/hostcheck.cpp
--- a/stark_mlwe_amd/csrc/hostcheck.cpp
+++ b/stark_mlwe_amd/csrc/hostcheck.cpp
@@ -31,7 +31,7 @@
     P->kc = host::make_kernel_consts(P->ref);
     P->dev.t = P->kc.t; P->dev.rf = P->kc.rf; P->dev.rp = P->kc.rp; P->dev.rc_full = P->kc.rc_full.data(); P->dev.rc_partial = P->kc.rc_partial.data();
     P->dev.lu = P->kc.lu.data(); P->dev.lu_pre = P->kc.lu_pre.data(); P->dev.row0 = P->kc.row0.data(); P->dev.sparse = P->kc.sparse.data(); P->dev.mds = P->kc.mds.data(); P->dev.mds_pre = P->kc.mds_pre.data(); P->dev.gamma = P->kc.gamma.data();
-    P->dev.lu29 = P->kc.lu29.data(); P->dev.lu_pre29 = P->kc.lu_pre29.data(); P->dev.row0_29 = P->kc.row0_29.data(); P->dev.sparse29 = P->kc.sparse29.data(); P->dev.gamma29 = P->kc.gamma29.data(); P->dev.mds29 = P->kc.mds29.data(); P->dev.mds_pre29 = P->kc.mds_pre29.data();
+    P->dev.lu29 = P->kc.lu29.data(); P->dev.lu_pre29 = P->kc.lu_pre29.data(); P->dev.row0_29 = P->kc.row0_29.data(); P->dev.sparse29 = P->kc.sparse29.data(); P->dev.gamma29 = P->kc.gamma29.data(); P->dev.mds29 = P->kc.mds29.data(); P->dev.mds_pre29 = P->kc.mds_pre29.data(); P->dev.rc_full29 = P->kc.rc_full29.data();
     P->dev.mds_frag = nullptr; P->dev.mds_pre_frag = nullptr; P->dev.blk8_efrag = nullptr; P->dev.blk8_lfrag = nullptr; P->dev.blk8_unit_frag = nullptr; P->dev.blk8_gfrag = nullptr;
     P->dev.chain_a = P->kc.chain_a.empty() ? nullptr : P->kc.chain_a.data(); P->dev.chain_g = P->kc.chain_g.empty() ? nullptr : P->kc.chain_g.data(); P->dev.chain_w = P->kc.chain_w.empty() ? nullptr : P->kc.chain_w.data();
 }
@@ -200,6 +200,31 @@
     }
     return 0;
 }
+int hc_mfma_finish_limbs(const int32_t* sums, size_t n, uint32_t* out) {
+    for (size_t s = 0; s < n; ++s) {
+        const int32_t* S = sums + 32 * s;
+        for (int c = 0; c < 32; ++c) if (S[c] >= (1 << 24) || S[c] <= -(1 << 24)) return -1;
+        int32_t lo[16], hi[16];
+        for (int reg = 0; reg < 16; ++reg) { const int row = (reg & 3) + 8 * (reg >> 2); lo[reg] = S[row]; hi[reg] = S[row + 4]; }
+        int64_t col[9]; for (int k = 0; k < 9; ++k) col[k] = 0;
+        mfma_fold_rows(col, lo, hi);
+        mfma_finish_limbs(col, out + 9 * s);
+    }
+    return 0;
+}
+int hc_sbox_lazy29(const uint32_t* l, const uint32_t* c, size_t n, uint64_t* out, uint64_t* colmax) {
+    for (size_t s = 0; s < n; ++s) {
+        const uint32_t* ls = l + 9 * s; const uint32_t* cs = c + 9 * s;
+        for (int i = 0; i < 9; ++i) if (ls[i] >= (i < 8 ? 1u << 29 : 1u << 24) || cs[i] >= (i < 8 ? 1u << 29 : 1u << 23)) return -1;
+        const fr_t z = sbox_lazy29(ls, cs);
+        Lazy29Wide wide; const fr29_t x5 = wide.pow5(ls, cs);
+        const fr_t zw = fr29_pack_reduce<PF>(x5.l);
+        if (colmax) { colmax[2 * s] = (uint64_t)wide.max_col; colmax[2 * s + 1] = (uint64_t)(wide.max_col >> 64); }
+        if ((wide.max_col >> 64) == 0 && memcmp(&z, &zw, sizeof(fr_t)) != 0) return -2;
+        st4(out + 4 * s, z);
+    }
+    return 0;
+}
 static int blk8_tile_sums(const int8_t* const* frag, const fr_t* xd, int K, int32_t* S) {
     for (int r = 0; r < 32; ++r) { int64_t acc = 0;
         for (int k = 0; k < K; ++k) for (int kh = 0; kh < 2; ++kh) { const int8_t* a = frag[k] + (size_t)(r + 32 * kh) * 16;
@@ -213,6 +238,13 @@
     int64_t col[9]; for (int k = 0; k < 9; ++k) col[k] = 0;
     mfma_fold_rows(col, lo, hi);
     return mfma_finish_cols(col);
+}
+static void blk8_finish_sums_limbs(const int32_t* S, uint32_t* l) {
+    int32_t lo[16], hi[16];
+    for (int reg = 0; reg < 16; ++reg) { const int row = (reg & 3) + 8 * (reg >> 2); lo[reg] = S[row]; hi[reg] = S[row + 4]; }
+    int64_t col[9]; for (int k = 0; k < 9; ++k) col[k] = 0;
+    mfma_fold_rows(col, lo, hi);
+    mfma_finish_limbs(col, l);
 }
 static int blk8_tile(const int8_t* const* frag, const fr_t* xd, int K, fr_t& out) { int32_t S[32]; const int rc = blk8_tile_sums(frag, xd, K, S); if (rc) return rc; out = blk8_finish_sums(S); return 0; }
 static std::atomic<int32_t> g_blk8_row23_max{0};
@@ -222,13 +254,20 @@
     if (t != 17 || k.blk8_efrag.empty() || k.blk8_gfrag.empty() || k.mds_frag.empty()) return -1;
     const int8_t* unit = k.blk8_lfrag.data() + k.blk8_lfrag.size() - 1024;
     std::vector<fr_t> st(t), xd(t), o(t);
-    auto full = [&](int r, const std::vector<int8_t>& F) -> int {
-        for (int j = 0; j < t; ++j) xd[j] = recode_signed(fr_pow5_r29<PF>(fr_add<PF>(st[j], k.rc_full[(size_t)r * t + j])));
-        for (int i = 0; i < t; ++i) { const int8_t* fr[17]; for (int e = 0; e < t; ++e) fr[e] = &F[((size_t)i * t + e) * 1024]; const int rc = blk8_tile(fr, xd.data(), t, o[i]); if (rc) return rc; }
-        st = o; return 0; };
+    auto sbox = [&](int r) { for (int j = 0; j < t; ++j) xd[j] = recode_signed(fr_pow5_r29<PF>(fr_add<PF>(st[j], k.rc_full[(size_t)r * t + j]))); };
+    auto product = [&](const std::vector<int8_t>& F, int next) -> int {
+        for (int i = 0; i < t; ++i) {
+            const int8_t* fr[17]; for (int e = 0; e < t; ++e) fr[e] = &F[((size_t)i * t + e) * 1024];
+            int32_t S[32]; const int rc = blk8_tile_sums(fr, xd.data(), t, S); if (rc) return rc;
+            if (next < 0) o[i] = blk8_finish_sums(S);
+            else { uint32_t l[9]; blk8_finish_sums_limbs(S, l); o[i] = recode_signed(sbox_lazy29(l, &k.rc_full29[((size_t)next * t + i) * 9])); }
+        }
+        if (next < 0) st = o; else xd = o;
+        return 0; };
     for (size_t s = 0; s < n; ++s) {
         for (int j = 0; j < t; ++j) st[j] = ld4(states + 4 * (s * t + j));
-        for (int r = 0; r < half; ++r) { const int rc = full(r, r == half - 1 ? k.mds_pre_frag : k.mds_frag); if (rc) return rc; }
+        sbox(0);
+        for (int r = 0; r < half; ++r) { const int rc = product(r == half - 1 ? k.mds_pre_frag : k.mds_frag, r == half - 1 ? -1 : r + 1); if (rc) return rc; }
         fr_t s0 = st[0], rec[17], y[8], yd[9], kx[23];
         for (int j = 1; j < t; ++j) rec[j] = recode_signed(st[j]);
         const int nb = k.rp / 8;
@@ -252,12 +291,14 @@
             for (int j = 1; j < t; ++j) {
                 const int8_t* fr[9]; for (int p2 = 0; p2 < 8; ++p2) fr[p2] = lf + ((size_t)(j - 1) * 8 + p2) * 1024; fr[8] = unit;
                 yd[8] = rec[j];
-                fr_t z; { const int rc = blk8_tile(fr, yd, 9, z); if (rc) return rc; }
-                if (b == nb - 1) st[j] = z; else rec[j] = recode_signed(z);
+                if (b == nb - 1) {
+                    int32_t S[32]; { const int rc = blk8_tile_sums(fr, yd, 9, S); if (rc) return rc; }
+                    uint32_t l[9]; blk8_finish_sums_limbs(S, l); xd[j] = recode_signed(sbox_lazy29(l, &k.rc_full29[((size_t)half * t + j) * 9]));
+                } else { fr_t z; { const int rc = blk8_tile(fr, yd, 9, z); if (rc) return rc; } rec[j] = recode_signed(z); }
             }
         }
-        st[0] = s0;
-        for (int r = half; r < k.rf; ++r) { const int rc = full(r, k.mds_frag); if (rc) return rc; }
+        xd[0] = recode_signed(fr_pow5_r29<PF>(fr_add<PF>(s0, k.rc_full[(size_t)half * t])));
+        for (int r = half; r < k.rf; ++r) { const int rc = product(k.mds_frag, r == k.rf - 1 ? -1 : r + 1); if (rc) return rc; }
         for (int j = 0; j < t; ++j) st4(states + 4 * (s * t + j), st[j]);
     }
     return 0;
@@ -268,6 +309,11 @@
     const size_t len = which == 0 ? k.blk8_efrag.size() : which == 1 ? k.blk8_lfrag.size() : which == 3 ? k.blk8_gfrag.size() : k.gamma8_29.size() * 4;
     if (out && len) memcpy(out, src, std::min(cap, len));
     return len;
+}
+size_t hc_rc_full29_table(void* h, uint32_t* out, size_t cap) {
+    const std::vector<uint32_t>& v = ((HcParams*)h)->kc.rc_full29;
+    if (out && !v.empty()) memcpy(out, v.data(), std::min(cap, v.size()) * 4);
+    return v.size();
 }
 int hc_blk8_finish_with_base(void* h, const int32_t* sums, const uint64_t* bases, size_t n, uint64_t* out) {
     HcParams* P = (HcParams*)h; if (P->kc.blk8_lfrag.empty()) return -3;
diff --git a/stark_mlwe_amd/csrc/mfma_digits.hpp b/stark_mlwe_amd/csrc/mfma_digits.hpp
--- a/stark_mlwe_amd/csrc/mfma_digits.hpp
+++ b/stark_mlwe_amd/csrc/mfma_digits.hpp
@@ -23,10 +23,9 @@
                 col[k] += pair * ((int64_t)1 << sh);
             }
 }
-FR_HD fr_t mfma_finish_cols(int64_t* col) {
+FR_HD void mfma_finish_limbs(int64_t* col, uint32_t* l) {
     typedef PallasFr PF;
     static_assert(fr_p29<PF>(4) < (1u << 10) && fr_p29<PF>(5) == 0 && fr_p29<PF>(6) == 0 && fr_p29<PF>(7) == 0 && fr_p29<PF>(8) == (1u << 22), "r = 2^254 + t with t below 2^126");
-    uint32_t l[9];
 #pragma unroll
     for (int k = 0; k < 8; ++k) { col[k + 1] += col[k] >> 29; l[k] = (uint32_t)col[k] & FR_M29; }
     const int64_t top = col[8];
@@ -38,9 +37,53 @@
     int32_t c32 = (int32_t)carry;
 #pragma unroll
     for (int i = 5; i < 9; ++i) { const int32_t d = (int32_t)l[i] + c32; if (i < 8) { l[i] = (uint32_t)d & FR_M29; c32 = d >> 29; } else l[8] = (uint32_t)d; }
+}
+FR_HD fr_t mfma_finish_cols(int64_t* col) {
+    typedef PallasFr PF;
+    uint32_t l[9];
+    mfma_finish_limbs(col, l);
     fr_t z = fr29_pack_reduce<PF>(l);
     fr_cond_sub<PF>(z.v, 0u);
     return z;
 }
+FR_HD fr_t sbox_lazy29(const uint32_t* l, const uint32_t* c) {
+    typedef PallasFr PF;
+    fr29_t u;
+#pragma unroll
+    for (int i = 0; i < 9; ++i) u.l[i] = l[i] + c[i];
+    const fr29_t x2 = fr29_sqr_mont<PF>(u), x4 = fr29_sqr_mont<PF>(x2), x5 = fr29_mul_mont<PF>(u, x4);
+    return fr29_pack_reduce<PF>(x5.l);
+}
+#if !defined(__HIP_DEVICE_COMPILE__)
+struct Lazy29Wide {
+    typedef unsigned __int128 u128;
+    u128 max_col = 0;
+    void mont(u128* w, uint32_t* l) {
+        typedef PallasFr PF;
+        for (int k = 0; k < 9; ++k) {
+            const u128 t = w[k]; if (t > max_col) max_col = t;
+            const uint32_t m = (0u - (uint32_t)t) & FR_M29;
+            w[k + 1] += (t + FR_M29) >> 29;
+            for (int j = 1; j < 9; ++j) if (fr_p29<PF>(j) != 0) w[k + j] += (u128)m * fr_p29<PF>(j);
+        }
+        u128 carry = 0;
+        for (int i = 0; i < 9; ++i) { const u128 v = w[9 + i] + carry; if (w[9 + i] > max_col) max_col = w[9 + i]; l[i] = i < 8 ? ((uint32_t)v & FR_M29) : (uint32_t)v; carry = v >> 29; }
+    }
+    fr29_t sqr(const fr29_t& a) {
+        u128 w[18]; for (int k = 0; k < 18; ++k) w[k] = 0;
+        for (int i = 0; i < 9; ++i) { w[2 * i] += (u128)a.l[i] * a.l[i]; for (int j = i + 1; j < 9; ++j) w[i + j] += (u128)a.l[i] * ((uint64_t)a.l[j] << 1); }
+        fr29_t r; mont(w, r.l); return r;
+    }
+    fr29_t mul(const fr29_t& a, const fr29_t& b) {
+        u128 w[18]; for (int k = 0; k < 18; ++k) w[k] = 0;
+        for (int i = 0; i < 9; ++i) for (int j = 0; j < 9; ++j) w[i + j] += (u128)a.l[i] * b.l[j];
+        fr29_t r; mont(w, r.l); return r;
+    }
+    fr29_t pow5(const uint32_t* l, const uint32_t* c) {
+        fr29_t u; for (int i = 0; i < 9; ++i) u.l[i] = l[i] + c[i];
+        const fr29_t x2 = sqr(u), x4 = sqr(x2); return mul(u, x4);
+    }
+};
+#endif
 
 }
diff --git a/stark_mlwe_amd/csrc/poseidon_pair.hpp b/stark_mlwe_amd/csrc/poseidon_pair.hpp
--- a/stark_mlwe_amd/csrc/poseidon_pair.hpp
+++ b/stark_mlwe_amd/csrc/poseidon_pair.hpp
@@ -88,8 +88,7 @@
                 col[k] += pair * ((int64_t)1 << sh);
             }
 }
-__device__ __forceinline__ fr_t mfma_finish_cols(int64_t* col) {
-    uint32_t l[9];
+__device__ __forceinline__ void mfma_finish_limbs(int64_t* col, uint32_t* l) {
 #pragma unroll
     for (int k = 0; k < 8; ++k) { col[k + 1] += col[k] >> 29; l[k] = (uint32_t)col[k] & FR_M29; }
     const int64_t top = col[8];
@@ -101,9 +100,32 @@
     int32_t c32 = (int32_t)carry;
 #pragma unroll
     for (int i = 5; i < 9; ++i) { const int32_t d = (int32_t)l[i] + c32; if (i < 8) { l[i] = (uint32_t)d & FR_M29; c32 = d >> 29; } else l[8] = (uint32_t)d; }
+}
+__device__ __forceinline__ fr_t mfma_finish_cols(int64_t* col) {
+    uint32_t l[9];
+#pragma unroll
+    for (int k = 0; k < 8; ++k) { col[k + 1] += col[k] >> 29; l[k] = (uint32_t)col[k] & FR_M29; }
+    const int64_t top = col[8];
+    const int32_t q1 = (int32_t)(top >> 22) - 1;
+    l[8] = ((uint32_t)top & ((1u << 22) - 1)) + (1u << 22);
+    int64_t carry = 0;
+#pragma unroll
+    for (int i = 0; i < 5; ++i) { const int64_t d = (int64_t)l[i] - (int64_t)q1 * (int64_t)fr_p29<PF>(i) + carry; l[i] = (uint32_t)d & FR_M29; carry = d >> 29; }
+    int32_t c32 = (int32_t)carry;
+#pragma unroll
+    for (int i = 5; i < 9; ++i) { const int32_t d = (int32_t)l[i] + c32; if (i < 8) { l[i] = (uint32_t)d & FR_M29; c32 = d >> 29; } else l[8] = (uint32_t)d; }
     fr_t z = fr29_pack_reduce<PF>(l);
     fr_cond_sub<PF>(z.v, 0u);
     return z;
+}
+__device__ __forceinline__ fr_t sbox_lazy29(const uint32_t* l, const uint32_t* __restrict__ c_) {
+    typedef const __attribute__((address_space(4))) uint32_t* cptr_t;
+    cptr_t c = (cptr_t)c_;
+    fr29_t u;
+#pragma unroll
+    for (int i = 0; i < 9; ++i) u.l[i] = l[i] + c[i];
+    const fr29_t x2 = fr29_sqr_mont<PF>(u), x4 = fr29_sqr_mont<PF>(x2), x5 = fr29_mul_mont<PF>(u, x4);
+    return fr29_pack_reduce<PF>(x5.l);
 }
 __device__ __forceinline__ void pair_apply_mds_mfma(const PairState& s, const void* frag) {
     constexpr int T = 17;
@@ -141,6 +163,51 @@
         for (int k = 0; k < 9; ++k) col[k] = 0;
         mfma_fold_rows(col, lo, hi);
         s.sto(i, mfma_finish_cols(col));
+    }
+    __syncthreads();
+}
+
+__device__ __forceinline__ void pair_mds_sbox_mfma(const PairState& s, const void* frag, const uint32_t* rc29, bool recode) {
+    constexpr int T = 17;
+    static_assert(fr_p29<PF>(4) < (1u << 10) && fr_p29<PF>(5) == 0 && fr_p29<PF>(6) == 0 && fr_p29<PF>(7) == 0 && fr_p29<PF>(8) == (1u << 22), "r = 2^254 + t with t below 2^126");
+    const int lane = s.lane, h = lane >> 5;
+    mfma_v4i b[T][2];
+#pragma unroll
+    for (int e = 0; e < T; ++e)
+#pragma unroll
+        for (int ct = 0; ct < 2; ++ct) { const uint4 u = s.st[(2 * e + h) * 64 + 32 * ct + (lane & 31)]; b[e][ct] = mfma_v4i{(int)u.x, (int)u.y, (int)u.z, (int)u.w}; }
+    __syncthreads();
+    const mfma_v4i* A = reinterpret_cast<const mfma_v4i*>(frag) + lane;
+#pragma unroll 1
+    for (int i = s.isY ? 1 : 0; i < T; i += 2) {
+        mfma_v16i acc[2];
+#pragma unroll
+        for (int ct = 0; ct < 2; ++ct)
+#pragma unroll
+            for (int r = 0; r < 16; ++r) acc[ct][r] = 0;
+        const mfma_v4i* Ai = A + (size_t)i * T * 64;
+#pragma unroll
+        for (int e = 0; e < T; ++e) {
+            const mfma_v4i a = Ai[(size_t)e * 64];
+#pragma unroll
+            for (int ct = 0; ct < 2; ++ct) acc[ct] = __builtin_amdgcn_mfma_i32_32x32x32_i8(a, b[e][ct], acc[ct], 0, 0, 0);
+        }
+        mfma_v16i lo, hi;
+#pragma unroll
+        for (int r = 0; r < 16; ++r) {
+            const auto sw = __builtin_amdgcn_permlane32_swap((unsigned)acc[0][r], (unsigned)acc[1][r], false, false);
+            lo[r] = (int)sw[0]; hi[r] = (int)sw[1];
+        }
+        int64_t col[9];
+#pragma unroll
+        for (int k = 0; k < 9; ++k) col[k] = 0;
+        mfma_fold_rows(col, lo, hi);
+        if (rc29) {
+            uint32_t l[9];
+            mfma_finish_limbs(col, l);
+            const fr_t y = sbox_lazy29(l, c29(rc29, i));
+            s.sto(i, recode ? recode_signed(y) : y);
+        } else s.sto(i, mfma_finish_cols(col));
     }
     __syncthreads();
 }
@@ -158,6 +225,17 @@
     __host__ __device__ static constexpr int ymail(int q) { return 17 + (q & 1); }
     __host__ __device__ static constexpr int hmail(int q) { return (q & 1) ? 19 : 0; }
 };
+__device__ __forceinline__ void mfma_post_cols(const mfma_v16i (&acc)[2], int64_t* col) {
+    mfma_v16i lo, hi;
+#pragma unroll
+    for (int r = 0; r < 16; ++r) {
+        const auto sw = __builtin_amdgcn_permlane32_swap((unsigned)acc[0][r], (unsigned)acc[1][r], false, false);
+        lo[r] = (int)sw[0]; hi[r] = (int)sw[1];
+    }
+#pragma unroll
+    for (int k = 0; k < 9; ++k) col[k] = 0;
+    mfma_fold_rows(col, lo, hi);
+}
 __device__ __forceinline__ fr_t mfma_post(const mfma_v16i (&acc)[2]) {
     mfma_v16i lo, hi;
 #pragma unroll
@@ -220,7 +298,7 @@
     b[Q][0] = blk8_b_of_slot(s, Blk8Cfg::ymail(Q), 0); b[Q][1] = blk8_b_of_slot(s, Blk8Cfg::ymail(Q), 1);
 }
 template <int NLX>
-__device__ __forceinline__ void blk8_lane_rows(const PairState& s, const Blk8Tabs& Tb, const mfma_v4i (&b)[8][2], bool last) {
+__device__ __forceinline__ void blk8_lane_rows(const PairState& s, const Blk8Tabs& Tb, const mfma_v4i (&b)[8][2], bool last, const uint32_t* rc29_next = nullptr, bool recode_next = true) {
     static_assert(NLX >= 1 && NLX <= 15, "shares");
     const int lane = s.lane;
     const int j0 = s.isY ? NLX + 1 : 1, j1 = s.isY ? 16 : NLX;
@@ -244,13 +322,17 @@
         const int jn = j < j1 ? j + 1 : j1;
 #pragma unroll
         for (int p = 0; p < 8; ++p) a[p] = (Tb.lfrag + ((size_t)(jn - 1) * 8 + p) * 64)[lane];
-        const fr_t z = mfma_post(acc);
-        s.sto(j, last ? z : recode_signed(z));
+        if (rc29_next) {
+            int64_t col[9]; uint32_t l[9];
+            mfma_post_cols(acc, col); mfma_finish_limbs(col, l);
+            const fr_t y = sbox_lazy29(l, c29(rc29_next, j));
+            s.sto(j, recode_next ? recode_signed(y) : y);
+        } else { const fr_t z = mfma_post(acc); s.sto(j, last ? z : recode_signed(z)); }
     }
     __syncthreads();
 }
 template <int NLX>
-__device__ __forceinline__ void pair_block8(const PairState& s, const Blk8Tabs& Tb, fr_t& s0, bool last) {
+__device__ __forceinline__ void pair_block8(const PairState& s, const Blk8Tabs& Tb, fr_t& s0, bool last, const uint32_t* rc29_next = nullptr, const fr_t* rc_next = nullptr, bool recode_next = true) {
     mfma_v4i b[8][2];
     if (!s.isY) {
         blk8_round_x<0>(s, Tb, s0, b); blk8_round_x<1>(s, Tb, s0, b); blk8_round_x<2>(s, Tb, s0, b); blk8_round_x<3>(s, Tb, s0, b);
@@ -262,7 +344,8 @@
         blk8_round_y<4>(s, Tb, b, a, g); blk8_round_y<5>(s, Tb, b, a, g); blk8_round_y<6>(s, Tb, b, a, g); blk8_round_y<7>(s, Tb, b, a, g);
     }
     __builtin_amdgcn_sched_barrier(0);
-    blk8_lane_rows<NLX>(s, Tb, b, last);
+    if (rc29_next && !s.isY) { const fr_t y = fr_pow5_r29<PF>(fr_add<PF>(s0, rc_next[0])); s.sto(0, recode_next ? recode_signed(y) : y); }
+    blk8_lane_rows<NLX>(s, Tb, b, last, rc29_next, recode_next);
 }
 
 template <int T>
@@ -274,12 +357,18 @@
     return fr_add<PF>(base, fr_wide29_reduce_lazy<PF>(u));
 }
 
-template <int T, bool BLK8 = false>
+template <int T, bool BLK8 = false, bool FUSE = BLK8>
 __device__ __forceinline__ fr_t pair_permute(const PairState& s, const PoseidonDev& P, bool only0, int r_begin = 0) {
     static_assert(!BLK8 || T == 17, "8-round blocks exist for t = 17");
+    static_assert(!FUSE || BLK8, "the fused hand-over belongs to the 8-round form");
     typedef PairCfg<T> Cfg;
     constexpr int NXD = Cfg::NXD, NXU = Cfg::NXU, W = 2 * T - 1;
     const int half = P.rf / 2;
+    if constexpr (FUSE) {
+        if (r_begin < half) pair_sbox_full<T, true>(s, P.rc_full + r_begin * T);
+        for (int r = r_begin; r < half; ++r)
+            pair_mds_sbox_mfma(s, (r == half - 1) ? P.mds_pre_frag : P.mds_frag, (r == half - 1) ? nullptr : c29(P.rc_full29, (size_t)(r + 1) * T), true);
+    } else
     for (int r = r_begin; r < half; ++r) {
         if constexpr (T == 17) { pair_sbox_full<T, true>(s, P.rc_full + r * T); pair_apply_mds_mfma(s, (r == half - 1) ? P.mds_pre_frag : P.mds_frag); }
         else { pair_sbox_full<T>(s, P.rc_full + r * T); pair_apply_lu<T>(s, (r == half - 1) ? P.lu_pre29 : P.lu29); }
@@ -295,7 +384,8 @@
             const Blk8Tabs Tb{reinterpret_cast<const mfma_v4i*>(P.blk8_efrag) + (size_t)b * 8 * 16 * 64, reinterpret_cast<const mfma_v4i*>(P.blk8_lfrag) + (size_t)b * 16 * 8 * 64,
                               reinterpret_cast<const mfma_v4i*>(P.blk8_unit_frag), reinterpret_cast<const mfma_v4i*>(P.blk8_gfrag) + (size_t)b * 28 * 64,
                               c29(P.sparse29, (size_t)(8 * b) * W), P.rc_partial + 8 * b};
-            pair_block8<Blk8Cfg::NLX>(s, Tb, s0, b == nb - 1);
+            if constexpr (FUSE) pair_block8<Blk8Cfg::NLX>(s, Tb, s0, b == nb - 1, b == nb - 1 ? c29(P.rc_full29, (size_t)half * T) : nullptr, P.rc_full + half * T, !(only0 && half == P.rf - 1));
+            else pair_block8<Blk8Cfg::NLX>(s, Tb, s0, b == nb - 1);
         }
     } else
     for (int b = 0; b < P.rp / 4; ++b) {
@@ -345,11 +435,14 @@
         }
         __syncthreads();
     }
-    if (!s.isY) s.sto(0, s0);
-    __syncthreads();
+    if constexpr (!FUSE) {
+        if (!s.isY) s.sto(0, s0);
+        __syncthreads();
+    }
     for (int r = half; r < P.rf; ++r) {
         const bool squeeze = only0 && r == P.rf - 1;
-        if constexpr (T == 17) { if (squeeze) pair_sbox_full<T>(s, P.rc_full + r * T); else pair_sbox_full<T, true>(s, P.rc_full + r * T); }
+        if constexpr (FUSE) {  }
+        else if constexpr (T == 17) { if (squeeze) pair_sbox_full<T>(s, P.rc_full + r * T); else pair_sbox_full<T, true>(s, P.rc_full + r * T); }
         else pair_sbox_full<T>(s, P.rc_full + r * T);
         if (squeeze) {
             const int j0 = s.isY ? Cfg::NX : 0, j1 = s.isY ? T : Cfg::NX;
@@ -362,7 +455,8 @@
             __syncthreads();
             return out;
         }
-        if constexpr (T == 17) pair_apply_mds_mfma(s, P.mds_frag); else pair_apply_lu<T>(s, P.lu29);
+        if constexpr (FUSE) pair_mds_sbox_mfma(s, P.mds_frag, r == P.rf - 1 ? nullptr : c29(P.rc_full29, (size_t)(r + 1) * T), !(only0 && r + 1 == P.rf - 1));
+        else if constexpr (T == 17) pair_apply_mds_mfma(s, P.mds_frag); else pair_apply_lu<T>(s, P.lu29);
     }
     return s.ld(0);
 }
@@ -416,7 +510,7 @@
             }
         }
         __syncthreads();
-        res = pair_permute<T, BLK8>(s, P, pidx + 1 == max_perm);
+        res = pair_permute<T, BLK8, false>(s, P, pidx + 1 == max_perm);
         __syncthreads();
     }
     if (live && !s.isY) stg(out + k0, res);
diff --git a/stark_mlwe_amd/csrc/poseidon_params.hpp b/stark_mlwe_amd/csrc/poseidon_params.hpp
--- a/stark_mlwe_amd/csrc/poseidon_params.hpp
+++ b/stark_mlwe_amd/csrc/poseidon_params.hpp
@@ -17,6 +17,7 @@
     const void* mds_frag; const void* mds_pre_frag;
     const uint32_t* chain_a; const uint32_t* chain_g; const uint32_t* chain_w;
     const void* blk8_efrag; const void* blk8_lfrag; const void* blk8_unit_frag; const void* blk8_gfrag;
+    const uint32_t* rc_full29;
 };
 
 }
```
